# schmeing/ReSeq

Measured on AMD Instinct MI355X. Metric: simulated read-pairs/sec (2x150 bp), higher is better.
Workload: dtype f64

## Files before the change

### include/reseq_amd.h

```cpp
#ifndef RESEQ_AMD_H
#define RESEQ_AMD_H

#include <stddef.h>
#include <stdint.h>

#ifdef __cplusplus
extern "C" {
#endif

typedef struct rsq_profile rsq_profile;
typedef struct rsq_ref rsq_ref;
typedef struct rsq_sim rsq_sim;

enum {
    RSQ_OK = 0,
    RSQ_EINVAL = -1,
    RSQ_EIO = -2,
    RSQ_ENODEV = -3,
    RSQ_EHIP = -4,
    RSQ_ENOSPC = -5,
    RSQ_ESTATE = -6
};

const char *rsq_last_error(void);
const char *rsq_last_warning(void);
const char *rsq_version(void);
int rsq_set_option(const char *name, int64_t value);
int rsq_get_option(const char *name, int64_t *value);
int rsq_device_count(void);

int rsq_profile_load(const char *path, rsq_profile **out);
int rsq_profile_is_reseq_archive(const char *path, int *yes);
int rsq_profile_load_reseq(const char *stats_path, const char *ipf_path, double ipf_precision_percent, rsq_profile **out);
int rsq_profile_archive_layout(const char *stats_path, const char *ipf_path, char *out, size_t cap, size_t *need);
int rsq_profile_save(const rsq_profile *p, const char *path);
int rsq_profile_save_reseq(const rsq_profile *p, const char *stats_path, const char *ipf_path, uint64_t creation_time);
void rsq_profile_free(rsq_profile *p);
int rsq_profile_change_error_rate(rsq_profile *p, double error_multiplier);
int rsq_profile_remove_substitution_errors(rsq_profile *p);
int rsq_profile_remove_indel_errors(rsq_profile *p);
int rsq_profile_max_read_length(const rsq_profile *p, uint32_t *out);
int rsq_profile_num_tiles(const rsq_profile *p, uint32_t *out);
int rsq_profile_max_len_deletion(const rsq_profile *p, uint32_t *out);
int rsq_profile_ref_seq_bias(const rsq_profile *p, double *out, size_t cap, size_t *n);

int rsq_ref_load_fasta(const char *path, rsq_ref **out);
int rsq_ref_replace_n(rsq_ref *r, uint64_t seed);
void rsq_ref_free(rsq_ref *r);
int rsq_ref_num_sequences(const rsq_ref *r, uint32_t *out);
int rsq_ref_sequence_length(const rsq_ref *r, uint32_t seq, uint32_t *out);
int rsq_ref_sequence_name(const rsq_ref *r, uint32_t seq, char *out, size_t cap);
int rsq_ref_write_fasta(const rsq_ref *r, const char *path);
int rsq_ref_read_variants(rsq_ref *r, const char *path);
int rsq_ref_num_alleles(const rsq_ref *r, uint32_t *out);
int rsq_ref_num_variants(const rsq_ref *r, uint32_t seq, uint32_t *out);
int rsq_ref_get_variant(const rsq_ref *r, uint32_t seq, uint32_t index, uint32_t *position, char *var_seq, size_t var_seq_cap, uint64_t allele_bits[2]);
int rsq_ref_get_codes(const rsq_ref *r, uint32_t seq, uint8_t *out, uint32_t len);

int rsq_sim_create(const rsq_profile *p, const rsq_ref *ref, int device, rsq_sim **out);
void rsq_sim_free(rsq_sim *s);
int rsq_sim_take_options(rsq_sim *s);

int rsq_sim_reference_sequence(rsq_sim *s, uint32_t seq, uint32_t start_pos, uint32_t frag_length, int reversed, int32_t first_variant_id, uint32_t first_variant_pos, uint32_t allele,
                               uint8_t *out, size_t cap);

int rsq_sim_prepare(rsq_sim *s, uint64_t seed, uint64_t num_read_pairs, double coverage, int ref_bias_mode, const char *record_base_identifier, void *stream);

int rsq_sim_prepare_plan(rsq_sim *s, uint64_t seed, uint64_t num_read_pairs, double coverage, int ref_bias_mode, const char *record_base_identifier);
int rsq_sim_bias_partials(rsq_sim *s, uint32_t block_lo, uint32_t block_hi, double *sums, double *maxes, size_t cap, size_t *n, void *stream);
int rsq_sim_prepare_normalization(rsq_sim *s, const double *sums, const double *maxes, size_t n);
int rsq_sim_prepare_sys_errors(rsq_sim *s, uint32_t block_lo, uint32_t block_hi, const uint32_t in_state[2], uint32_t out_state[2], void *stream);
int rsq_sim_prepare_finish(rsq_sim *s);

int rsq_sim_read_methylation(rsq_sim *s, const char *path);

int rsq_sim_set_ref_bias_file(rsq_sim *s, const char *path);
int rsq_sim_get_ref_seq_bias(const rsq_sim *s, double *out, size_t n);

typedef struct {
    uint64_t total_pairs;
    uint64_t adapter_only_pairs;
    uint32_t total_blocks;
    uint32_t n_coverage_groups;
    uint32_t insert_to;
    uint32_t sys_chain_passes;
    double bias_normalization;
} rsq_sim_info;
int rsq_sim_get_info(const rsq_sim *s, rsq_sim_info *out);
int rsq_sim_get_fill_plan(const rsq_sim *s, uint32_t *quality_quads, uint32_t *image_tiles, uint32_t *image_bytes);
int rsq_sim_export_reference(rsq_sim *s, const char *path);
int rsq_sim_get_sequence_lengths(const rsq_sim *s, uint32_t *out, size_t cap, uint32_t *n_sequences);
int rsq_sim_import_reference(rsq_sim *s, const char *path);
int rsq_sim_specialize(rsq_sim *s, int kind, int *specialized);
int rsq_set_kernel_cache_dir(const char *path);
int rsq_profile_compile_read_kernel(const rsq_profile *p, int kind, int with_variants, int binned, const char *arch, const char *out_path, size_t *code_bytes, double *seconds);

int rsq_sim_get_thresholds(const rsq_sim *s, double *out, size_t n);
int rsq_sim_get_norm_by_len(const rsq_sim *s, double *out, size_t n);
int rsq_sim_set_normalization(rsq_sim *s, double bias_normalization, const double *thresholds, size_t n);
int rsq_sim_get_sys_errors(const rsq_sim *s, int reverse_strand, uint32_t seq, uint8_t *dom_out, uint8_t *rate_out, uint32_t len);
int rsq_sim_get_adapter_sys_errors(const rsq_sim *s, int template_segment, uint32_t adapter, uint8_t *dom_out, uint8_t *rate_out, uint32_t len);

int rsq_sim_create_sys_error_profile(rsq_sim *s, uint64_t seed, const char *path, void *stream);
int rsq_sim_read_sys_errors(rsq_sim *s, const char *path);

typedef struct {
    uint32_t seq, start, len;
    uint16_t dup;
    uint8_t strand, pad;
    uint32_t block, number;
} rsq_fragment;

int rsq_sim_block_weights(const rsq_sim *s, double *weights, size_t cap, uint32_t *n_blocks);
int rsq_partition_blocks(uint32_t total_blocks, uint32_t workers, const double *weights, uint32_t *bounds);

int rsq_sim_job_generate(rsq_sim *s, uint32_t block_lo, uint32_t block_hi, uint32_t batch_blocks, uint64_t *n_pairs, uint64_t *r1_bytes, uint64_t *r2_bytes, void *stream);
int rsq_sim_job_write(rsq_sim *s, const char *r1_path, uint64_t r1_offset, const char *r2_path, uint64_t r2_offset, uint32_t threads_per_file);
int rsq_sim_job_compress(rsq_sim *s, uint64_t *r1_bytes, uint64_t *r2_bytes);

size_t rsq_gzip_bound(size_t text_len);
size_t rsq_gzip_eof_member(char *out, size_t cap);
int rsq_sim_gzip_keep_code(rsq_sim *s, int keep);
int rsq_sim_gzip_device(rsq_sim *s, const char *text_dev, size_t text_len, char *out_dev, size_t out_cap, size_t *out_len, void *stream);
int rsq_sim_job_read(rsq_sim *s, int file, uint64_t at, size_t bytes, char *dst_dev, void *stream);
int rsq_sim_job_free(rsq_sim *s);
// ... 50 lines not shown
```

### reseq_amd/api.py

```python
import ctypes as C
import os

import numpy as np

_HERE = os.path.dirname(os.path.abspath(__file__))
LIB_PATH = os.path.join(_HERE, "libreseq_amd.so")

RSQ_OK, RSQ_EINVAL, RSQ_EIO, RSQ_ENODEV, RSQ_EHIP, RSQ_ENOSPC, RSQ_ESTATE = 0, -1, -2, -3, -4, -5, -6

FRAGMENT_DTYPE = np.dtype([("seq", "<u4"), ("start", "<u4"), ("len", "<u4"), ("dup", "<u2"), ("strand", "u1"),
                           ("allele", "u1"), ("block", "<u4"), ("number", "<u4")])


class SimInfo(C.Structure):
    _fields_ = [("total_pairs", C.c_uint64), ("adapter_only_pairs", C.c_uint64), ("total_blocks", C.c_uint32),
                ("n_coverage_groups", C.c_uint32), ("insert_to", C.c_uint32), ("sys_chain_passes", C.c_uint32),
                ("bias_normalization", C.c_double)]


class RsqError(RuntimeError):
    def __init__(self, code, message):
        super().__init__(f"rsq error {code}: {message}")
        self.code = code


_vp, _u64, _u32, _sz = C.c_void_p, C.c_uint64, C.c_uint32, C.c_size_t
_pp = C.POINTER(C.c_void_p)
_psz = C.POINTER(C.c_size_t)
SYMBOLS = {
    "rsq_last_error": (C.c_char_p, []),
    "rsq_version": (C.c_char_p, []),
    "rsq_set_option": (C.c_int, [C.c_char_p, C.c_int64]),
    "rsq_get_option": (C.c_int, [C.c_char_p, C.POINTER(C.c_int64)]),
    "rsq_device_count": (C.c_int, []),
    "rsq_profile_load": (C.c_int, [C.c_char_p, _pp]),
    "rsq_profile_load_reseq": (C.c_int, [C.c_char_p, C.c_char_p, C.c_double, _pp]),
    "rsq_profile_is_reseq_archive": (C.c_int, [C.c_char_p, C.POINTER(C.c_int)]),
    "rsq_profile_save": (C.c_int, [C.c_void_p, C.c_char_p]),
    "rsq_profile_save_reseq": (C.c_int, [C.c_void_p, C.c_char_p, C.c_char_p, C.c_uint64]),
    "rsq_profile_archive_layout": (C.c_int, [C.c_char_p, C.c_char_p, C.c_char_p, C.c_size_t, C.POINTER(C.c_size_t)]),
    "rsq_last_warning": (C.c_char_p, []),
    "rsq_profile_free": (None, [_vp]),
    "rsq_profile_change_error_rate": (C.c_int, [_vp, C.c_double]),
    "rsq_profile_remove_substitution_errors": (C.c_int, [_vp]),
    "rsq_profile_remove_indel_errors": (C.c_int, [_vp]),
    "rsq_profile_max_read_length": (C.c_int, [_vp, C.POINTER(_u32)]),
    "rsq_profile_num_tiles": (C.c_int, [_vp, C.POINTER(_u32)]),
    "rsq_profile_max_len_deletion": (C.c_int, [_vp, C.POINTER(_u32)]),
    "rsq_profile_ref_seq_bias": (C.c_int, [_vp, _vp, _sz, _psz]),
    "rsq_ref_sequence_name": (C.c_int, [_vp, _u32, C.c_char_p, _sz]),
    "rsq_ref_load_fasta": (C.c_int, [C.c_char_p, _pp]),
    "rsq_ref_replace_n": (C.c_int, [_vp, _u64]),
    "rsq_ref_free": (None, [_vp]),
    "rsq_ref_num_sequences": (C.c_int, [_vp, C.POINTER(_u32)]),
    "rsq_ref_sequence_length": (C.c_int, [_vp, _u32, C.POINTER(_u32)]),
    "rsq_ref_write_fasta": (C.c_int, [_vp, C.c_char_p]),
    "rsq_ref_read_variants": (C.c_int, [_vp, C.c_char_p]),
    "rsq_ref_num_alleles": (C.c_int, [_vp, C.POINTER(_u32)]),
    "rsq_ref_num_variants": (C.c_int, [_vp, _u32, C.POINTER(_u32)]),
    "rsq_ref_get_variant": (C.c_int, [_vp, _u32, _u32, C.POINTER(_u32), C.c_char_p, _sz, C.POINTER(_u64)]),
    "rsq_ref_get_codes": (C.c_int, [_vp, _u32, _vp, _u32]),
    "rsq_sim_create": (C.c_int, [_vp, _vp, C.c_int, _pp]),
    "rsq_sim_free": (None, [_vp]),
    "rsq_sim_take_options": (C.c_int, [_vp]),
    "rsq_sim_prepare": (C.c_int, [_vp, _u64, _u64, C.c_double, C.c_int, C.c_char_p, _vp]),
    "rsq_sim_prepare_plan": (C.c_int, [_vp, _u64, _u64, C.c_double, C.c_int, C.c_char_p]),
    "rsq_sim_bias_partials": (C.c_int, [_vp, _u32, _u32, _vp, _vp, C.c_size_t, C.POINTER(C.c_size_t), _vp]),
    "rsq_sim_prepare_normalization": (C.c_int, [_vp, _vp, _vp, C.c_size_t]),
    "rsq_sim_prepare_sys_errors": (C.c_int, [_vp, _u32, _u32, _vp, _vp, _vp]),
    "rsq_sim_prepare_finish": (C.c_int, [_vp]),
    "rsq_sim_get_info": (C.c_int, [_vp, C.POINTER(SimInfo)]),
    "rsq_sim_get_fill_plan": (C.c_int, [_vp, C.POINTER(_u32), C.POINTER(_u32), C.POINTER(_u32)]),
    "rsq_sim_specialize": (C.c_int, [_vp, C.c_int, C.POINTER(C.c_int)]),
    "rsq_sim_export_reference": (C.c_int, [_vp, C.c_char_p]),
    "rsq_sim_block_weights": (C.c_int, [_vp, _vp, _sz, C.POINTER(_u32)]),
    "rsq_partition_blocks": (C.c_int, [_u32, _u32, _vp, _vp]),
    "rsq_sim_reference_sequence": (C.c_int, [_vp, _u32, _u32, _u32, C.c_int, C.c_int32, _u32, _u32, _vp, _sz]),
    "rsq_sim_job_read": (C.c_int, [_vp, C.c_int, _u64, _sz, _vp, _vp]),
    "rsq_dev_pwrite": (C.c_int, [C.c_int, _vp, _sz, C.c_char_p, _u64]),
    "rsq_sim_get_sequence_lengths": (C.c_int, [_vp, _vp, _sz, C.POINTER(_u32)]),
    "rsq_sim_import_reference": (C.c_int, [_vp, C.c_char_p]),
    "rsq_set_kernel_cache_dir": (C.c_int, [C.c_char_p]),
    "rsq_profile_compile_read_kernel": (C.c_int, [_vp, C.c_int, C.c_int, C.c_int, C.c_char_p, C.c_char_p, C.POINTER(C.c_size_t), C.POINTER(C.c_double)]),
    "rsq_sim_get_thresholds": (C.c_int, [_vp, _vp, _sz]),
    "rsq_sim_get_norm_by_len": (C.c_int, [_vp, _vp, _sz]),
    "rsq_sim_set_normalization": (C.c_int, [_vp, C.c_double, _vp, _sz]),
    "rsq_sim_get_sys_errors": (C.c_int, [_vp, C.c_int, _u32, _vp, _vp, _u32]),
    "rsq_sim_get_adapter_sys_errors": (C.c_int, [_vp, C.c_int, _u32, _vp, _vp, _u32]),
    "rsq_sim_create_sys_error_profile": (C.c_int, [_vp, _u64, C.c_char_p, _vp]),
    "rsq_sim_read_sys_errors": (C.c_int, [_vp, C.c_char_p]),
    "rsq_sim_set_ref_bias_file": (C.c_int, [_vp, C.c_char_p]),
    "rsq_sim_read_methylation": (C.c_int, [_vp, C.c_char_p]),
    "rsq_sim_get_ref_seq_bias": (C.c_int, [_vp, _vp, _sz]),
    "rsq_sim_pairs": (C.c_int, [_vp, _u32, _u32, _vp, _sz, _psz, _vp, _sz, _psz, C.POINTER(_u64), _vp, _sz, _vp]),
    "rsq_sim_job_generate": (C.c_int, [_vp, _u32, _u32, _u32, C.POINTER(_u64), C.POINTER(_u64), C.POINTER(_u64), _vp]),
    "rsq_sim_job_write": (C.c_int, [_vp, C.c_char_p, _u64, C.c_char_p, _u64, _u32]),
    "rsq_sim_job_compress": (C.c_int, [_vp, C.POINTER(_u64), C.POINTER(_u64)]),
    "rsq_gzip_bound": (C.c_size_t, [C.c_size_t]),
    "rsq_gzip_eof_member": (C.c_size_t, [C.c_char_p, C.c_size_t]),
    "rsq_sim_gzip_keep_code": (C.c_int, [_vp, C.c_int]),
    "rsq_sim_gzip_device": (C.c_int, [_vp, _vp, C.c_size_t, _vp, C.c_size_t, C.POINTER(C.c_size_t), _vp]),
    "rsq_sim_job_free": (C.c_int, [_vp]),
    "rsq_sim_adapter_only_pairs": (C.c_int, [_vp, _u64, _u64, _vp, _sz, _psz, _vp, _sz, _psz, _vp]),
    "rsq_sim_error_model": (C.c_int, [_vp, _u64, _u64, _u32, _vp, _vp, _vp, _vp, _vp, _vp, _vp, _u32, _vp, _vp, _vp, _vp, _u32, _vp]),
    "rsq_sim_error_model_fastq": (C.c_int, [_vp, _u64, _u64, _u32, _vp, _vp, _vp, _vp, _vp, _vp, _vp, _vp, C.c_size_t, C.POINTER(C.c_size_t), _vp]),
    "rsq_sim_error_model_file": (C.c_int, [_vp, C.c_char_p, C.c_char_p, _vp, C.POINTER(_u64), C.POINTER(_u64)]),
    "rsq_fasta_count_records": (C.c_int, [C.c_char_p, _u64, _u64, _u32, C.POINTER(_u64), C.POINTER(_u64)]),
    "rsq_sim_error_model_fasta": (C.c_int, [_vp, _u64, _vp, C.c_size_t, C.c_int, _vp, C.c_size_t, C.POINTER(C.c_size_t), C.POINTER(_u64), C.POINTER(C.c_size_t), _vp]),
    "rsq_sim_last_kernel_ms": (C.c_int, [_vp, C.c_char_p, C.POINTER(C.c_double)]),
    "rsq_sim_last_kernel_launches": (C.c_int, [_vp, C.c_char_p, C.POINTER(_u32)]),
    "rsq_dev_alloc": (C.c_int, [C.c_int, _sz, _pp]),
    "rsq_dev_free": (C.c_int, [C.c_int, _vp]),
    "rsq_dev_upload": (C.c_int, [C.c_int, _vp, _vp, _sz]),
    "rsq_dev_download": (C.c_int, [C.c_int, _vp, _vp, _sz]),
    "rsq_host_alloc": (C.c_int, [_sz, _pp]),
    "rsq_host_free": (C.c_int, [_vp]),
    "rsq_stream_create": (C.c_int, [C.c_int, _pp]),
    "rsq_stream_destroy": (C.c_int, [C.c_int, _vp]),
    "rsq_dev_copy_on": (C.c_int, [C.c_int, _vp, _vp, _sz, C.c_int, _vp]),
}

_lib = None


def lib():
    global _lib
    if _lib is None:
        if not os.path.exists(LIB_PATH):
            raise ImportError(f"{LIB_PATH} is missing: build it with `python -c 'import __graft_entry__ as g; g.build()'` "
                              "(make -C reseq_amd/csrc); reseq_amd has no CPU fallback")
        L = C.CDLL(LIB_PATH)
        for name, (res, args) in SYMBOLS.items():
            fn = getattr(L, name)
            fn.restype = res
            fn.argtypes = args
        _lib = L
    return _lib


def use_library(path):
    global LIB_PATH, _lib
    if _lib is not None:
        raise RuntimeError("the library is already loaded")
    LIB_PATH = os.path.abspath(path)


def set_option(name, value):
    _check(lib().rsq_set_option(name.encode(), int(value)))


def get_option(name):
    v = C.c_int64(0)
    _check(lib().rsq_get_option(name.encode(), C.byref(v)))
    return v.value


def archive_layout(stats_path, ipf_path=None):
    need = C.c_size_t(0)
    ipf = ipf_path.encode() if ipf_path else None
    _check(lib().rsq_profile_archive_layout(str(stats_path).encode(), ipf, None, 0, C.byref(need)))
    buf = C.create_string_buffer(need.value)
    _check(lib().rsq_profile_archive_layout(str(stats_path).encode(), ipf, buf, need.value, C.byref(need)))
    return buf.value.decode(errors="replace")


def gzip_eof_member():
    buf = C.create_string_buffer(32)
    n = lib().rsq_gzip_eof_member(buf, 32)
    return buf.raw[:n]


def partition_blocks(total_blocks, workers, weights=None):
    w = np.ascontiguousarray(np.ones(total_blocks) if weights is None else weights, dtype=np.float64)
    if w.size != total_blocks:
        raise ValueError("one weight per block")
    bounds = np.zeros(workers + 1, np.uint32)
    _check(lib().rsq_partition_blocks(total_blocks, workers, w.ctypes.data, bounds.ctypes.data))
    return [(int(bounds[r]), int(bounds[r + 1])) for r in range(workers)]


def dev_pwrite(device, src_ptr, nbytes, path, offset):
    _check(lib().rsq_dev_pwrite(device, C.c_void_p(src_ptr), nbytes, os.fsencode(path), offset))


def set_kernel_cache_dir(path):
    _check(lib().rsq_set_kernel_cache_dir((path or "").encode()))


def last_warning():
    return lib().rsq_last_warning().decode(errors="replace")


def _check(rc):
    if rc != RSQ_OK:
        raise RsqError(rc, lib().rsq_last_error().decode(errors="replace"))


def device_count():
    n = lib().rsq_device_count()
    if n < 0:
        raise RsqError(n, lib().rsq_last_error().decode())
    return n


class Profile:

    def __init__(self, path, ipf_path=None, ipf_precision=5.0):
        self.h = C.c_void_p()
        if ipf_path is None and ipf_precision == 5.0:
            _check(lib().rsq_profile_load(os.fsencode(path), C.byref(self.h)))
        else:
            _check(lib().rsq_profile_load_reseq(os.fsencode(path), os.fsencode(ipf_path) if ipf_path else None, ipf_precision, C.byref(self.h)))
        self.warning = lib().rsq_last_warning().decode()

    def save(self, path):
        _check(lib().rsq_profile_save(self.h, os.fsencode(path)))

    def save_reseq(self, stats_path, ipf_path=None, creation_time=0):
        _check(lib().rsq_profile_save_reseq(self.h, os.fsencode(stats_path), os.fsencode(ipf_path) if ipf_path else None, int(creation_time)))

    def compile_read_kernel(self, kind=0, with_variants=False, binned=False, arch="gfx950", out_path=None):
        n, t = C.c_size_t(0), C.c_double(0.0)
        _check(lib().rsq_profile_compile_read_kernel(self.h, kind, int(with_variants), int(binned), arch.encode(), os.fsencode(out_path) if out_path else None, C.byref(n), C.byref(t)))
        return n.value, t.value

    def change_error_rate(self, multiplier):
        _check(lib().rsq_profile_change_error_rate(self.h, multiplier))

    def remove_substitution_errors(self):
        _check(lib().rsq_profile_remove_substitution_errors(self.h))

    def remove_indel_errors(self):
        _check(lib().rsq_profile_remove_indel_errors(self.h))

    def max_read_length(self):
        v = C.c_uint32()
        _check(lib().rsq_profile_max_read_length(self.h, C.byref(v)))
        return v.value

    def close(self):
        if self.h:
            lib().rsq_profile_free(self.h)
            self.h = C.c_void_p()


def load_profile(path, ipf_path=None, ipf_precision=5.0):
    archive = C.c_int(0)
    lib().rsq_profile_is_reseq_archive(os.fsencode(path), C.byref(archive))
    if not archive.value:
        return Profile(path)
    p = Profile.__new__(Profile)
    p.h = C.c_void_p()
    _check(lib().rsq_profile_load_reseq(os.fsencode(path), os.fsencode(ipf_path) if ipf_path else None, float(ipf_precision), C.byref(p.h)))
    p.warning = lib().rsq_last_warning().decode()
    return p


class Reference:

    def __init__(self, fasta_path, replace_n_seed=None):
        self.h = C.c_void_p()
        _check(lib().rsq_ref_load_fasta(os.fsencode(fasta_path), C.byref(self.h)))
        if replace_n_seed is not None:
            _check(lib().rsq_ref_replace_n(self.h, replace_n_seed))

    def num_sequences(self):
        v = C.c_uint32()
        _check(lib().rsq_ref_num_sequences(self.h, C.byref(v)))
        return v.value

    def sequence_length(self, i):
        v = C.c_uint32()
        _check(lib().rsq_ref_sequence_length(self.h, i, C.byref(v)))
        return v.value

    def sequence_name(self, i):
        buf = C.create_string_buffer(1 << 16)
        _check(lib().rsq_ref_sequence_name(self.h, i, buf, len(buf)))
        return buf.value.decode()

    def read_variants(self, path):
        _check(lib().rsq_ref_read_variants(self.h, str(path).encode()))
        n = _u32()
        _check(lib().rsq_ref_num_alleles(self.h, C.byref(n)))
        return n.value

    def variants(self, seq):
        n = _u32()
        _check(lib().rsq_ref_num_variants(self.h, seq, C.byref(n)))
        out = []
        for i in range(n.value):
            pos, buf, bits = _u32(), C.create_string_buffer(1 << 16), (_u64 * 2)()
            _check(lib().rsq_ref_get_variant(self.h, seq, i, C.byref(pos), buf, len(buf), bits))
            out.append((pos.value, buf.value.decode(), bits[0] | (bits[1] << 64)))
        return out

    def write_fasta(self, path):
        _check(lib().rsq_ref_write_fasta(self.h, str(path).encode()))

    def codes(self, i):
        out = np.zeros(self.sequence_length(i), np.uint8)
        _check(lib().rsq_ref_get_codes(self.h, i, out.ctypes.data, len(out)))
        return out

    def close(self):
        if self.h:
            lib().rsq_ref_free(self.h)
            self.h = C.c_void_p()


class ErrorModelFileOptions(C.Structure):
    _fields_ = [("read_threads", C.c_uint32), ("block_kb", C.c_uint32), ("batch_blocks", C.c_uint32), ("keep_text", C.c_uint32), ("from_", C.c_uint64), ("to", C.c_uint64), ("first_record", C.c_uint64),
                ("progress", C.c_void_p), ("user", C.c_void_p), ("trace", C.c_char_p), ("trace_cap", C.c_size_t)]


def count_fasta_records(path, from_=0, to=0, threads=0):
    n, first = _u64(0), _u64(0)
    _check(lib().rsq_fasta_count_records(os.fsencode(path), from_, to, threads, C.byref(n), C.byref(first)))
    return n.value, first.value


class DeviceArray:

    def __init__(self, device, nbytes):
        self.device, self.nbytes = device, int(nbytes)
        self.ptr = C.c_void_p()
# ... 319 lines not shown
```

### reseq_amd/csrc/rsq_core.h

```cpp
#pragma once
#include "rsq_types.h"
#if !defined(__HIPCC_RTC__)
#include <math.h>
#endif

namespace rsq {

struct Words {
    uint32_t w0, w1, w2, w3;
};


RSQ_HD Words philox(uint64_t seed, uint32_t c0, uint32_t c1, uint32_t c2, uint32_t c3) {
    uint32_t k0 = (uint32_t)seed, k1 = (uint32_t)(seed >> 32);
#pragma unroll
    for (int r = 0; r < 10; ++r) {
        const uint64_t p0 = (uint64_t)0xD2511F53u * c0, p1 = (uint64_t)0xCD9E8D57u * c2;
        const uint32_t hi0 = (uint32_t)(p0 >> 32), lo0 = (uint32_t)p0, hi1 = (uint32_t)(p1 >> 32), lo1 = (uint32_t)p1;
        c0 = hi1 ^ c1 ^ k0;
        c1 = lo1;
        c2 = hi0 ^ c3 ^ k1;
        c3 = lo0;
        k0 += 0x9E3779B9u;
        k1 += 0xBB67AE85u;
// ... 620 lines not shown

    template <class Tab, class Src, class Out>
    RSQ_HD bool step(const DevSim &S, const Tab &tab, const Stream &st, const Src &src, Out &out) {
        if (!advance(S, st)) return false;
        iterate(S, tab, st, src, out);
        return true;
    }
    RSQ_HD bool in_template() const { return phase == kTemplate && par.read_pos < par.read_length && org_pos < org_len; }
    template <bool TEMPLATE_PART = false, class Tab, class Src, class Out>
    RSQ_HD void iterate(const DevSim &S, const Tab &tab, const Stream &st, const Src &src, Out &out) {
        const bool tail = !TEMPLATE_PART && phase == kTail, from_template = TEMPLATE_PART || phase == kTemplate;
        const DevAdapters &ad = S.adapters[seg];
        const uint32_t it = par.iteration;
        const Words w = st.step(2u + it);
        typename Tab::Sum prob_sum;
        uint32_t indel = 0, org_base = 0;
        if (!tail) {
            const uint32_t idx_i[3] = {par.indel_pos, par.read_pos, par.gc_seq};
            indel = tab.draw_indel(par.previous_indel_type * 6u + par.base_call, idx_i, w.w0, prob_sum);
            if (0 == prob_sum) indel = 0;
            org_base = from_template ? src.base(org_pos) : (uint32_t)ad.seqs[adapter_a0 + org_pos];
        }
        const uint32_t qi = tbase + org_base;
        const bool regular = !tail && 0 == indel, deletion = !tail && 1 == indel;
        uint32_t dom_error = 0;
        if (regular) {
            const uint32_t se = from_template ? src.sys_base(org_pos) : (uint32_t)ad.sys[adapter_a0 + org_pos];
            dom_error = se & 0xFFu;
            par.error_rate = se >> 8;
        } else if (deletion) {
            par.error_rate = (from_template ? src.sys_deleted(org_pos) : (uint32_t)ad.sys[adapter_a0 + org_pos]) >> 8;
        }
        uint32_t q = 0;
        if (!deletion) {
            const uint32_t idx_q[4] = {par.seq_qual, par.qual, par.read_pos, par.error_rate};
            q = tab.draw_quality(qi, idx_q, w.w1, prob_sum);
            if (0 == prob_sum) {
                if (regular) q = par.read_pos ? par.last_written_qual : tab.quality(qi).max_value;
                else if (tail) q = par.read_pos ? par.last_written_qual : q;
                else q = par.qual;
            }
        }
        uint32_t put_base = 0, op_code = 0;
        char element = 0;
        const bool insertion = !tail && indel > 1u;
        if (regular) {
            par.qual = q;
            const uint32_t idx_b[4] = {par.qual, par.read_pos, par.num_errors, par.error_rate};
            uint32_t call = tab.draw_base_call(qi * 5u + dom_error, idx_b, w.w2, prob_sum);
            if (0 == prob_sum) call = org_base;
            par.base_call = call;
            put_base = call;
            element = from_template ? 'M' : 'S';
            if (call != org_base) ++par.num_errors;
        } else if (deletion) {
            op_code = 1u;
            element = 'D';
        } else if (tail) {
            par.qual = q;
            put_base = pos_tail < tail_length ? 0u : discrete_draw(S.overrun_cp, 4, u32_to_unit(w.w3));
            ++pos_tail;
        } else {
            put_base = indel - 2u;
            op_code = 2u;
            element = 'I';
        }
        if (element) {
            const uint32_t is_indel = deletion || insertion ? 1u : 0u;
            n_indels += is_indel;
            par.num_errors += is_indel;
            if (element == cg.element) {
                ++cg.length;
                par.indel_pos += is_indel;
            } else {
                cg.flush();
                cg.element = element;
                cg.length = 1;
                par.indel_pos = is_indel;
                par.previous_indel_type = deletion ? 1u : 0u;
            }
            if (!insertion) ++org_pos;
        }
        if (!deletion) {
            out.put(par.read_pos, put_base, q + RSQ_SIM(S, phred_offset));
            par.last_written_qual = q;
            ++par.read_pos;
        }
        if (!tail) out.op(it, op_code);
        par.iteration = it + 1u;
    }

    RSQ_HD void finalize(ReadMeta &meta) const {
        meta.read_len = (uint16_t)par.read_length;
        meta.num_errors = (uint16_t)par.num_errors;
        meta.n_iter_m = (uint16_t)iter_m;
        meta.n_iter_s = (uint16_t)(par.iteration - iter_m - hard_clip);
        meta.hard_clip = (uint16_t)hard_clip;
        meta.tile_id = (uint16_t)tile_id;
        meta.cigar_chars = (uint16_t)cg.chars;
        meta.plain = n_indels ? 0u : 1u;
    }
};

template <class Tab, class Src, class Out>
RSQ_HD void fill_read(const DevSim &S, const Tab &tab, const Stream &st, uint32_t seg, uint32_t tile_id, uint32_t fragment_length, const Src &src, Out &out,
                      ReadMeta &meta) {
    ReadMachine m;
    m.init(S, tab, st, seg, tile_id, fragment_length, src);
    while (m.step(S, tab, st, src, out)) {}
    m.finalize(meta);
}

}
```

### reseq_amd/csrc/rsq_format.h

```cpp
#pragma once
#include "rsq_reads.h"

namespace rsq {

#if RSQ_DEVICE_BUILD
#ifndef RSQ_BIN_KEYS_LDS
#define RSQ_BIN_KEYS_LDS 4096
#endif
constexpr uint32_t kBinKeysLds = RSQ_BIN_KEYS_LDS;
constexpr uint32_t kBinItemsPerThread = 16, kBinBlock = 256;

__device__ inline void bin_count_key(uint32_t key, bool valid, uint32_t n_keys, uint32_t *hist, uint32_t *s_hist) {
    if (n_keys <= kBinKeysLds) {
        for (uint32_t k = threadIdx.x; k < n_keys; k += blockDim.x) s_hist[k] = 0;
        __syncthreads();
        if (valid) atomicAdd(&s_hist[key], 1u);
        __syncthreads();
        for (uint32_t k = threadIdx.x; k < n_keys; k += blockDim.x)
            if (s_hist[k]) atomicAdd(&hist[k], s_hist[k]);
    } else if (valid) atomicAdd(&hist[key], 1u);
}
__global__ void __launch_bounds__(kBinBlock) k_pair_tiles(DevSim S, const Fragment *frags, const FragmentVar *fvars, uint64_t n_pairs, uint64_t adapter_only_first, uint16_t *key_of,
                                                         uint32_t *hist) {
    __shared__ uint32_t s_hist[kBinKeysLds];
// ... 96 lines not shown
    const uint64_t i = (uint64_t)blockIdx.x * blockDim.x + threadIdx.x;
    if (i >= n) return;
    const uint32_t seg = segs[i] ? 1u : 0u, fl = frag_len[i];
    if (fl < range.lo[seg] || fl >= range.hi[seg]) atomicMin(first_bad, (uint32_t)i);
}
__global__ void k_record_flags(const uint8_t *segs, uint64_t n, uint32_t *flags) {
    const uint64_t i = (uint64_t)blockIdx.x * blockDim.x + threadIdx.x;
    if (i < n) flags[i] = segs[i] ? 1u : 0u;
}
__global__ void k_record_partition(const uint8_t *segs, uint64_t n, const uint64_t *ones_before, uint32_t *rec_index, uint32_t *rec_count) {
    const uint64_t i = (uint64_t)blockIdx.x * blockDim.x + threadIdx.x;
    const uint32_t n1 = (uint32_t)ones_before[n], n0 = (uint32_t)n - n1;
    if (i == 0) {
        rec_count[0] = n0;
        rec_count[1] = n1;
    }
    if (i >= n) return;
    const uint32_t before = (uint32_t)ones_before[i];
    if (segs[i]) rec_index[n0 + before] = (uint32_t)i;
    else rec_index[(uint32_t)i - before] = (uint32_t)i;
}

__global__ void __launch_bounds__(256) k_methylation_templates(DevSim S, const Fragment *frags, uint64_t n_pairs, RawLayout raw) {
    const uint64_t r = (uint64_t)blockIdx.x * blockDim.x + threadIdx.x;
    if (r >= 2u * n_pairs) return;
    const uint32_t seg = r >= n_pairs ? 1u : 0u;
    convert_template(S, frags[r - seg * n_pairs], seg, raw.templates + r * raw.template_words, raw.template_words);
}

__global__ void __launch_bounds__(256) k_variant_templates(DevSim S, const Fragment *frags, const FragmentVar *fvars, uint64_t n_pairs, RawLayout raw) {
    const uint64_t r = (uint64_t)blockIdx.x * blockDim.x + threadIdx.x;
    if (r >= 2u * n_pairs) return;
    const uint32_t seg = r >= n_pairs ? 1u : 0u;
    const uint64_t pair = r - seg * n_pairs;
    variant_template(S, frags[pair], fvars[pair], seg, raw.templates + r * raw.template_words, raw.template_words);
}

#ifndef RSQ_FORMAT_RECORDS
#define RSQ_FORMAT_RECORDS 16
#endif
constexpr uint32_t kFormatRecords = RSQ_FORMAT_RECORDS, kFormatLdsMax = 16u * 1024u, kFormatLdsMin = 1024u;
RSQ_HD uint32_t format_lds_bytes(uint64_t record_bytes) {
    const uint64_t want = (kFormatRecords * record_bytes + 16u + 127u) & ~(uint64_t)127u;
    return (uint32_t)(want < kFormatLdsMin ? kFormatLdsMin : want > kFormatLdsMax ? kFormatLdsMax : want);
}
__global__ void __launch_bounds__(256) k_max_size(const uint32_t *sizes, uint64_t n, uint32_t *longest) {
    uint32_t m = 0;
    for (uint64_t i = (uint64_t)blockIdx.x * blockDim.x + threadIdx.x; i < n; i += (uint64_t)gridDim.x * blockDim.x) m = max(m, sizes[i]);
    for (uint32_t d = 32; d; d >>= 1) m = max(m, (uint32_t)__shfl_xor((int)m, (int)d, 64));
    if ((threadIdx.x & 63u) == 0 && m) atomicMax(longest, m);
}
template <bool PERM>
__global__ void __launch_bounds__(64) k_format_write(DevSim S, NameTable names, const Fragment *frags, uint64_t n_pairs, uint64_t adapter_only_first, RawLayout raw,
                                                    const uint64_t *offsets0, const uint64_t *offsets1, char *dst0, char *dst1, uint64_t cap0, uint64_t cap1,
                                                    const FragmentVar *fvars, const uint32_t *perm, uint32_t lds_bytes) {
    extern __shared__ __attribute__((aligned(16))) char s_text[];
    const uint32_t lane = threadIdx.x, seg = blockIdx.y, rec = lane & (kFormatRecords - 1u), part = lane / kFormatRecords;
    constexpr uint32_t kLineParts = 32u / kFormatRecords;
    const bool is_qual = part >= kLineParts;
    const uint32_t sub = part % kLineParts;
    const uint64_t first = (uint64_t)blockIdx.x * kFormatRecords;
    if (first >= n_pairs) return;
    const uint64_t *offsets = seg ? offsets1 : offsets0;
    char *dst = seg ? dst1 : dst0;
    if (offsets[n_pairs] > (seg ? cap1 : cap0)) return;
    const uint64_t last = first + kFormatRecords < n_pairs ? first + kFormatRecords : n_pairs;
    const uint64_t row = first + rec;
    const bool active = row < last;
    const uint64_t pair = PERM ? (active ? perm[row] : 0u) : row;
    const uint64_t g_begin = PERM ? (active ? offsets[pair] : 0u) : offsets[first], g_end = PERM ? (active ? offsets[pair + 1u] : 0u) : offsets[last];
    const uint32_t skew = (uint32_t)((uint64_t)(uintptr_t)(dst + g_begin) & 15u), bytes = (uint32_t)(g_end - g_begin);
    const uint32_t kSlot = (lds_bytes / kFormatRecords) & ~15u;
    const bool through_lds = PERM ? __all(skew + bytes <= kSlot) != 0 : skew + bytes <= lds_bytes;
    ReadMeta m;
    Fragment f;
    FragmentVar fv;
    uint64_t r = 0;
    if (active) {
        r = (uint64_t)seg * n_pairs + row;
        m = raw.meta[r];
        if (frags) f = frags[pair];
        if (frags && fvars) fv = fvars[pair];
    }
    const WordColumn seq = raw.seq_of(r), qual = raw.qual_of(r), ops = raw.ops_of(r);
    const uint64_t ao_number = adapter_only_first + pair + 1u;
    if (!through_lds) {
        if (active && part == 0u) format_record(S, names, frags != nullptr, f, ao_number, m, seq, qual, ops, dst + offsets[pair], frags && fvars, fv);
        return;
    }
    const uint32_t slot_at = PERM ? rec * kSlot : 0u;
    if (active) {
        RSQ_LDS char *rec_text = (RSQ_LDS char *)s_text + slot_at + skew + (PERM ? 0u : (uint32_t)(offsets[pair] - g_begin));
        const uint32_t header = (uint32_t)(offsets[pair + 1u] - offsets[pair]) - 2u * m.read_len - 4u;
        const uint32_t all_words = (m.read_len + 3u) >> 2, per = (all_words + kLineParts - 1u) / kLineParts;
        const uint32_t first_word = sub * per, line_at = header + (is_qual ? m.read_len + 3u : 0u);
        const uint32_t part_at = part == 0u ? 0u : line_at + (4u * first_word < m.read_len ? 4u * first_word : m.read_len);
        WordSinkT<RSQ_LDS char *> t(rec_text + part_at);
        if (part == 0u) format_header(S, names, frags != nullptr, f, ao_number, m, ops, t, frags && fvars, fv);
        format_line_part(is_qual ? qual : seq, m.read_len, is_qual, first_word, per, sub == kLineParts - 1u, t);
        t.finish();
    }
    __syncthreads();
    const uint32_t lo = skew, hi = skew + bytes;
    char *g_chunk0 = dst + g_begin - skew;
    const char *s_from = s_text + slot_at;
    for (uint32_t c = (PERM ? part : lane) * 16u; c < hi; c += (PERM ? 64u / kFormatRecords : 64u) * 16u) {
        if (c >= lo && c + 16u <= hi) {
            *reinterpret_cast<uint4 *>(g_chunk0 + c) = *reinterpret_cast<const uint4 *>(s_from + c);
        } else {
            for (uint32_t b = c < lo ? lo : c; b < c + 16u && b < hi; ++b) g_chunk0[b] = s_from[b];
        }
    }
}

#endif

}
```

### reseq_amd/csrc/rsq_pack.h

```cpp
#pragma once
#include <math.h>
#include <stdio.h>
#include <stdlib.h>
#include <string.h>
#include <errno.h>
#include <fcntl.h>
#include <unistd.h>

#include <algorithm>
#include <string>
#include <vector>

#include <atomic>
#include <exception>
#include <mutex>
#include <thread>

#include "rsq_host.h"
#include "rsq_chains.h"
#include "rsq_sieve.h"
#include "rsq_reads.h"

namespace rsq {

// ... 339 lines not shown
        auto need_rate = [&](uint32_t rows_q, uint32_t rows_b) {
            return (uint64_t)4 * Ti * odd_stride((uint64_t)rows_q * plan.slot_q) + (uint64_t)20 * Ti * odd_stride((uint64_t)rows_b * plan.slot_b);
        };
        const uint32_t ring_stride = 4 * Ti * plan.slot_q;
        need += (uint64_t)kFillWavesMax * kRingRows * ring_stride;
        if (need + need_rate(1, 1) > budget) return false;
        uint32_t rq = 1, rb = 1;
        while (rq < std::min(rate_rows_q, kLdsRateRowsFirst) && need + need_rate(rq + 1, 1) <= budget) ++rq;
        const bool stage_b2 = need + need_b2 + need_rate(rq, 1) <= budget;
        if (stage_b2) need += need_b2;
        const bool stage_i0 = need + need_i0 + need_rate(rq, 1) <= budget;
        if (stage_i0) need += need_i0;
        while (rb < std::min(rate_rows_b, kLdsRateRowsFirst) && need + need_rate(rq, rb + 1) <= budget) ++rb;
        while (rq < rate_rows_q && need + need_rate(rq + 1, rb) <= budget) ++rq;
        while (rb < rate_rows_b && need + need_rate(rq, rb + 1) <= budget) ++rb;
        plan.img_tiles = Ti;
        plan.binned = (Ti < T || opt.image_tiles == 1) ? 1u : 0u;
        plan.par0_words = par0_words;
        plan.par0_indel_bytes = par0_indel_bytes;
        plan.desc_words = desc_words;
        plan.ring_stride = ring_stride;
        plan.rate_rows_q = rq;
        plan.rate_rows_b = rb;
        plan.q.values = desc_words * 4u;
        plan.b.values = plan.q.values + 4 * Ti * plan.slot_q;
        plan.i.values = plan.b.values + 20 * Ti * plan.slot_b;
        uint32_t at = desc_words + values_words;
        plan.q.lds = at, plan.q.lds_rows = rows_q, plan.q.lds_stride = stride_q, at += (uint32_t)need_q;
        plan.b.lds = at, plan.b.lds_rows = rows_b, plan.b.lds_stride = stride_b, at += (uint32_t)need_b;
        plan.b.lds2 = stage_b2 ? at : kNoLds;
        plan.b.lds2_stride = stride_b2;
        if (stage_b2) at += (uint32_t)need_b2;
        plan.i.lds = stage_i0 ? at : kNoLds;
        plan.i.lds_rows = rows_i;
        plan.i.lds_stride = stride_i;
        if (stage_i0) at += (uint32_t)need_i0;
        plan.ring_off = at;
        plan.q3_off = plan.ring_off + kFillWavesMax * kRingRows * plan.ring_stride;
        plan.q3_stride = odd_stride((uint64_t)plan.rate_rows_q * plan.slot_q);
        plan.b3_stride = odd_stride((uint64_t)plan.rate_rows_b * plan.slot_b);
        plan.b3_off = plan.q3_off + 4 * Ti * plan.q3_stride;
        plan.total_words = plan.b3_off + 20 * Ti * plan.b3_stride;
        plan.mask = plan.quads_q;
        return true;
    };
    plan.img_tiles = T;
    if (screenable && opt.fill_mode != 0) {
        const bool per_tile_first = opt.image_tiles == 1 && T > 1;
        if (!(per_tile_first && plan_image(1)) && !plan_image(T) && !(T > 1 && plan_image(1)))
            s.plan_note = "the read kernels' table image does not fit the " + std::to_string(kLdsBudgetBytes / 1024u) +
                          " KiB of local memory even for one tile: every per-base draw runs in double precision from device memory (several times slower)";
    } else if (!screenable && opt.fill_mode != 0)
        s.plan_note = "the profile's tables are outside what the screened single-precision draws are built for (more than " + std::to_string(4u * kQualityQuads[4]) +
                      " quality values, or more than 8 base-call / indel outcomes): every per-base draw runs in double precision from device memory (several times slower)";
    if ((plan.desc_words | plan.q3_off | plan.b3_off | plan.ring_off | plan.ring_stride | plan.slot_q | plan.slot_b | plan.slot_i | plan.q.off32 | plan.b.off32 | plan.i.off32 |
         (plan.mask ? plan.q.lds | plan.b.lds | (plan.b.lds2 != kNoLds ? plan.b.lds2 : 0u) | (plan.i.lds != kNoLds ? plan.i.lds : 0u) : 0u)) & 3u)
        throw Error("internal: LDS rows must start on 16-byte boundaries");
    if (opt.trace_plan)
        fprintf(stderr, "[rsq] LDS image: mask %u, %u of %u tiles per image, %u words (%u KiB), desc %u, quality slot %u, rate rows %u / %u, q3 %u b3 %u, ring %u x %u, b2 %d i0 %d\n", plan.mask,
                plan.img_tiles, T, plan.total_words, plan.total_words / 256, plan.desc_words, plan.slot_q, plan.rate_rows_q, plan.rate_rows_b, plan.q3_off, plan.b3_off, plan.ring_off,
                plan.ring_stride, (int)(plan.b.lds2 != kNoLds), (int)(plan.i.lds != kNoLds));
    s.dev.lds = plan;
    s.dev.quality = up.put(quality);
    s.dev.seq_quality = up.put(seq_quality);
    s.dev.base_call = up.put(base_call);
    s.dev.dom_error = up.put(dom_error);
    s.dev.error_rate = up.put(error_rate);
    s.dev.indels = up.put(indels);
    par0.resize(((par0.size() + 3u) & ~(size_t)3u) + (size_t)plan.par0_words * 4u + 16u, 0);
    pool.push_back(0.0);
    pool.push_back(0.0);
    pool32.resize(pool32.size() + 8, 0.f);
    s.dev.pool = up.put(pool);
    s.dev.pool32 = up.put(pool32);
    s.dev.par0 = up.put(par0);
    s.host_pool = pool;
    s.host_par0 = par0;
    s.host_dom_error = dom_error;
    s.host_error_rate = error_rate;
}

inline uint32_t effective_fill_mask(uint32_t plan_mask, int forced) { return forced == 0 ? 0u : plan_mask; }

inline void pack_profile(SimState &s, Uploader &up) {
    const Profile &p = s.prof;
    DevSim &d = s.dev;
    d.n_tiles = p.n_tiles();
    d.phred_offset = p.phred_offset;
    d.max_len_deletion = p.max_len_deletion;
    d.reset_distance = p.reset_distance;
    d.tile_cp = up.put(discrete_cp(p.tile_abundance.data(), p.tile_abundance.size()));
    d.tiles = up.put(p.tiles);
    s.rmax = 0;
    uint32_t max_adapter = 0;
    for (int seg = 0; seg < 2; ++seg) {
        const HostAdapters &a = p.adapters[seg];
        DevAdapters &da = d.adapters[seg];
        da.n = a.n();
        da.seqs = up.put(a.seqs);
        da.seq_ptr = up.put(a.seq_ptr);
        da.adapter_cp = up.put(discrete_cp(a.significant.data(), a.significant.size()));
        std::vector<double> cut_cp;
        for (uint32_t i = 0; i < a.n(); ++i) {
            std::vector<double> cp = discrete_cp(a.cut.data() + a.cut_ptr[i], a.cut_ptr[i + 1] - a.cut_ptr[i]);
            cp.resize(a.cut_ptr[i + 1] - a.cut_ptr[i]);
            cut_cp.insert(cut_cp.end(), cp.begin(), cp.end());
            max_adapter = std::max(max_adapter, a.seq_ptr[i + 1] - a.seq_ptr[i]);
        }
        cut_cp.push_back(1.0);
        da.cut_cp = up.put(cut_cp);
        da.cut_ptr = up.put(a.cut_ptr);
        da.cut_from = up.put(a.cut_from);
        s.adapter_sys[seg] = up.put(std::vector<uint16_t>(a.seqs.size() + 1, 0));
        da.sys = s.adapter_sys[seg];

        const Vect<uint64_t> &rl = p.read_lengths[seg];
        DevReadLengths &dr = d.read_lengths[seg];
        if (rl.v.empty()) throw Error("profile has no read lengths");
        dr.fixed = rl.v.size() == 1 ? (uint32_t)rl.from : 0u;
        dr.to = (uint32_t)rl.to();
        dr.row_first = (uint32_t)p.rl_by_fl[seg].from;
        dr.rows = (uint32_t)p.rl_by_fl[seg].row_ptr.size() - 1;
        dr.row_ptr = up.put(p.rl_by_fl[seg].row_ptr);
        dr.row_from = up.put(p.rl_by_fl[seg].row_from);
        dr.values = up.put(p.rl_by_fl[seg].values);
        s.rmax = std::max(s.rmax, dr.to - 1);
    }
    d.polya_cp = up.put(discrete_cp(p.polya.v.data(), p.polya.v.size()));
    d.polya_n = (uint32_t)p.polya.v.size();
    d.polya_from = (uint32_t)p.polya.from;
    std::vector<double> ocp = discrete_cp(p.overrun_bases, 4);
    for (int i = 0; i < 4; ++i) d.overrun_cp[i] = ocp[i];
    d.insert_from = (uint32_t)std::max<uint64_t>(1, p.insert_lengths.from);
    s.insert_lengths_from = p.insert_lengths.from;
    if (p.insert_lengths.to() > 65536) throw Error("insert lengths above 65535 are not supported (fragment lengths are 16-bit fields of the sieve's records)");
    d.insert_to = (uint32_t)p.insert_lengths.to();
    std::vector<uint64_t> il(d.insert_to + 1, 0);
    std::vector<double> ilb(d.insert_to + 1, 0.0), gcb(101, 0.0);
    for (uint32_t i = 0; i < d.insert_to; ++i) {
        il[i] = p.insert_lengths[i];
        ilb[i] = p.insert_lengths_bias[i];
    }
    for (uint32_t i = 0; i < 101; ++i) gcb[i] = p.gc_bias[i];
    d.insert_lengths = up.put(il);
    d.insert_lengths_bias = up.put(ilb);
    d.gc_bias = up.put(gcb);
    d.sur_bias = up.put(p.sur_bias);
    d.dispersion[0] = p.dispersion[0];
    d.dispersion[1] = p.dispersion[1];

    s.max_adapter = max_adapter;
    s.read_stride = (s.rmax + 15u) & ~15u;
    const uint32_t max_iter = 2u * s.rmax + p.max_len_deletion + max_adapter + 4u;
    s.ops_stride = (max_iter + 15u) / 16u;
}

inline int variants_mode_for(const Variants &v) {
    if (v.num_alleles > kMaxDevAlleles) throw Error("variants: more than " + std::to_string(kMaxDevAlleles) + " alleles");
    if (v.num_alleles > 8) return 2;
    for (const std::vector<Variant> &seq : v.by_seq)
        for (const Variant &x : seq)
            if (x.var_seq.size() != 1) return 2;
    return 1;
}

inline void allele_maps_of_sequence(const std::vector<Variant> &vars, const std::vector<uint8_t> &codes, uint32_t num_alleles, const std::string &name,
                                    std::vector<AlleleVar> &out, std::vector<uint32_t> &ptr) {
    auto is_gc_code = [](uint8_t c) { return c == 1 || c == 2; };
    for (uint32_t a = 0; a < num_alleles; ++a) {
        int32_t shift = 0, gc = 0;
        int64_t last_pos = -1;
// ... 1202 lines not shown
```

### reseq_amd/csrc/rsq_reads.h

```cpp
#pragma once
#include "rsq_core.h"
#include "rsq_variants.h"
#include "rsq_text.h"

namespace rsq {

struct ReadOut {
    WordColumn seq, qual, ops;
    uint32_t cur_word, cur_index;
    uint32_t seq_word, qual_word, n_put;
    RSQ_HD void put(uint32_t pos, uint32_t base, uint32_t qual_char) {
        const uint32_t sh = (pos & 3u) * 8u;
        seq_word |= base << sh;
        qual_word |= qual_char << sh;
        n_put = pos + 1u;
        if ((pos & 3u) == 3u) {
            seq.at(pos >> 2) = seq_word;
            qual.at(pos >> 2) = qual_word;
            seq_word = qual_word = 0;
        }
    }
    RSQ_HD void op(uint32_t it, uint32_t code) {
        const uint32_t wi = it >> 4;
        if (wi != cur_index) {
            ops.at(cur_index) = cur_word;
            cur_word = 0;
            cur_index = wi;
        }
        cur_word |= code << ((it & 15u) * 2u);
    }
    RSQ_HD void finish() {
        ops.at(cur_index) = cur_word;
        if (n_put & 3u) {
            seq.at(n_put >> 2) = seq_word;
            qual.at(n_put >> 2) = qual_word;
        }
    }
};
RSQ_HD ReadOut make_read_out(const WordColumn &seq, const WordColumn &qual, const WordColumn &ops) { return ReadOut{seq, qual, ops, 0u, 0u, 0u, 0u, 0u}; }

struct RawLayout {
    uint32_t *seq, *qual;
    uint32_t *ops;
    ReadMeta *meta;
    uint64_t pitch;
    uint64_t *templates;
    uint32_t template_words;
    const uint32_t *order;
    RSQ_HD uint64_t item_of(uint64_t row) const { return order ? order[row] : row; }
    RSQ_HD WordColumn seq_of(uint64_t r) const { return WordColumn{seq + r, pitch}; }
    RSQ_HD WordColumn qual_of(uint64_t r) const { return WordColumn{qual + r, pitch}; }
    RSQ_HD WordColumn ops_of(uint64_t r) const { return WordColumn{ops + r, pitch}; }
    RSQ_HD ReadOut out_of(uint64_t r) const { return make_read_out(seq_of(r), qual_of(r), ops_of(r)); }
};

struct FragmentSrc {
    const uint64_t *words;
    uint64_t word_off;
    uint32_t first;
    uint32_t len;
    bool reverse;
    const uint16_t *sys_;
    const uint64_t *converted;
    const uint32_t *gc_prefix;
    mutable uint32_t held_word = 0xFFFFFFFFu, held_sys = 0xFFFFFFFFu;
    mutable uint64_t word = 0, sys4 = 0;
    RSQ_HD uint64_t template_word(const uint64_t *from, uint32_t index) const {
        if (index != held_word) {
            held_word = index;
            word = from[index];
        }
        return word;
    }
    RSQ_HD uint32_t org_len() const { return len; }
    RSQ_HD uint32_t ref(uint32_t k) const {
        const uint32_t pos = reverse ? first - 1u - k : first + k, b = (uint32_t)(template_word(words + word_off, pos >> 5) >> ((pos & 31u) * 2u)) & 3u;
        return reverse ? 3u - b : b;
    }
    RSQ_HD uint32_t base(uint32_t k) const { return converted ? (uint32_t)(template_word(converted, k >> 5) >> ((k & 31u) * 2u)) & 3u : ref(k); }
    RSQ_HD uint32_t sys_base(uint32_t k) const {
        if ((k >> 2) != held_sys) {
            held_sys = k >> 2;
#if defined(__HIP_DEVICE_COMPILE__)
            sys4 = *reinterpret_cast<const uint64_t __attribute__((aligned(2))) *>(sys_ + (k & ~3u));
#else
            memcpy(&sys4, sys_ + (k & ~3u), 8);
#endif
        }
        return (uint32_t)(sys4 >> ((k & 3u) * 16u)) & 0xFFFFu;
    }
    RSQ_HD uint32_t sys_deleted(uint32_t k) const { return sys_base(k); }
    RSQ_HD void totals(uint32_t n, uint32_t &gc, uint32_t &rate_sum) const {
        if (!converted && !gc_prefix) return template_totals_loop(*this, n, gc, rate_sum);
        if (converted) gc += ref_gc_count(converted, 0, 0, n);
        else gc += reverse ? ref_gc_count_prefix(words, gc_prefix, word_off, first - n, first) : ref_gc_count_prefix(words, gc_prefix, word_off, first, first + n);
        rate_sum += rate_total(n);
    }
    RSQ_HD uint32_t rate_total(uint32_t n) const {
        struct __attribute__((packed, aligned(2))) Eight {
            uint64_t a, b;
        };
        uint32_t sum = 0;
        for (uint32_t k = 0; k < n; k += 8u) {
            Eight e;
#if defined(__HIP_DEVICE_COMPILE__)
            e = *reinterpret_cast<const Eight *>(sys_ + k);
#else
            memcpy(&e, sys_ + k, 16);
#endif
            const uint32_t left = n - k;
            if (left < 8u) {
                if (left <= 4u) {
                    e.b = 0;
                    if (left < 4u) e.a &= (1ull << (16u * left)) - 1ull;
                } else e.b &= (1ull << (16u * (left - 4u))) - 1ull;
            }
            const uint64_t kHigh = 0x00FF00FF00FF00FFull, kAdd = 0x0001000100010001ull;
            sum += (uint32_t)((((e.a >> 8) & kHigh) * kAdd) >> 48) + (uint32_t)((((e.b >> 8) & kHigh) * kAdd) >> 48);
        }
        return sum;
    }
};

struct MethView {
    const uint32_t *first, *second;
    const double *rate;
    uint32_t n, stride;
    RSQ_HD double rate_of(int32_t region) const { return rate[(size_t)region * stride]; }
};
RSQ_HD MethView meth_view(const DevSim &S, uint32_t seq, uint32_t allele = 0) {
    const uint32_t off = S.meth_ptr[seq];
    return MethView{S.meth_first + off, S.meth_second + off, S.meth_rate + (size_t)off * S.num_alleles + allele, S.meth_ptr[seq + 1] - off, S.num_alleles};
}
RSQ_HD uint32_t meth_start_index(const MethView &m, uint32_t pos) {
    uint32_t lo = 0, hi = m.n;
    while (lo < hi) {
// ... 669 lines not shown
struct FillBins {
    const uint32_t *perm;
    const uint32_t *bin_first;
    const uint32_t *bin_count;
    const uint32_t *chunk_ptr;
    uint32_t *next_chunk;
    uint32_t *workers;
    uint32_t n_bins;
    const Fragment *frags;
    const FragmentVar *fvars;
};
constexpr uint32_t kSchedWords = 8;

struct PairStream {
    uint32_t c0, c1, c2, strand;
};
RSQ_HD PairStream pair_stream(const Fragment *f, uint32_t sub, uint64_t adapter_only_number) {
    if (f) return PairStream{f->start, f->seq | (sub << 22), f->len | ((uint32_t)f->dup << 16), f->strand};
    return PairStream{(uint32_t)adapter_only_number, 0xFFFFFFFFu, (uint32_t)(adapter_only_number >> 32), 0u};
}

#if RSQ_DEVICE_BUILD
template <uint32_t MASK>
__device__ RSQ_LDS float *fill_stage_image(const DevSim &S, float *lds_image, uint32_t qbase) {
    RSQ_LDS float *img = (RSQ_LDS float *)lds_image;
    if (MASK) {
        lds_stage_descriptors(S, img, qbase, threadIdx.x, blockDim.x);
        __syncthreads();
        lds_stage_rows(S, img, qbase, threadIdx.x, blockDim.x);
        __syncthreads();
    }
    return img;
}
template <uint32_t MASK, class Src>
__device__ void fill_wave_reads(const DevSim &S, RSQ_LDS float *img, uint32_t qbase, uint32_t seg, bool active, const Stream &st, uint32_t tile, uint32_t fragment_length,
                                const Src &src, ReadOut &out, ReadMeta &meta) {
    ReadMachine m;
    if constexpr (MASK == 0) {
        const GlobalTables tab{S};
        if (active) {
            m.init(S, tab, st, seg, tile, fragment_length, src);
            while (m.step(S, tab, st, src, out)) {}
        }
    } else {
        const uint32_t lane = threadIdx.x & 63u, n_items = lds_ring_items(S);
        RSQ_LDS float *ring = img + RSQ_PLAN(S, ring_off) + (threadIdx.x >> 6) * kRingRows * RSQ_PLAN(S, ring_stride);
        ScreenTables<MASK> tab{S, img, qbase, ring, 0u};
        m.idle();
        if (active) m.init(S, tab, st, seg, tile, fragment_length, src);
        const RingItem mine = lds_ring_item(S, qbase, lane < n_items ? lane : 0u);
        Quad ahead = lane < n_items ? lds_ring_load(S, mine, 0u) : zero_quad();
        auto begin_step = [&](uint32_t t) {
            if (lane < n_items) {
                lds_ring_store(S, mine, ring, t, ahead);
                ahead = lds_ring_load(S, mine, t + 1u);
            }
            for (uint32_t item = lane + 64u; item < n_items; item += 64u) lds_ring_stage(S, qbase, ring, t, item);
            __builtin_amdgcn_wave_barrier();
            tab.t = t;
            const uint64_t lagging = __builtin_amdgcn_ballot_w64(m.phase != ReadMachine::kDone && t - m.par.read_pos > kRingLag);
            tab.demand = 0xFFFFFFFFu;
            if (lagging) {
                const uint32_t p = __builtin_amdgcn_readlane(m.par.read_pos, __builtin_ctzll(lagging));
                if (lane < n_items) lds_ring_stage_demand(S, mine, ring, p);
                for (uint32_t item = lane + 64u; item < n_items; item += 64u) lds_ring_stage_demand(S, lds_ring_item(S, qbase, item), ring, p);
                __builtin_amdgcn_wave_barrier();
                tab.demand = p;
            }
        };
        uint32_t t = 0;
        for (; !RSQ_ANY(!m.in_template()); ++t) {
            begin_step(t);
            m.template iterate<true>(S, tab, st, src, out);
            __builtin_amdgcn_wave_barrier();
        }
        for (; RSQ_ANY(m.phase != ReadMachine::kDone); ++t) {
            begin_step(t);
            m.step(S, tab, st, src, out);
            __builtin_amdgcn_wave_barrier();
        }
    }
    if (active) {
        m.finalize(meta);
        out.finish();
    }
}

template <uint32_t MASK, class Chunk>
__device__ void fill_binned_loop(const DevSim &S, float *lds_image, const FillBins &bins, Chunk &&chunk) {
    RSQ_LDS float *img = (RSQ_LDS float *)lds_image;
    RSQ_LDS uint32_t *sched = reinterpret_cast<RSQ_LDS uint32_t *>(img + (MASK ? RSQ_PLAN(S, total_words) : 0u));
    const uint32_t lane = threadIdx.x & 63u;
    if (threadIdx.x == 0) sched[1] = 0xFFFFFFFFu;
    for (bool first_choice = true;; first_choice = false) {
        if (threadIdx.x < 64u) {
            uint64_t best = 0;
            if (first_choice) {
                const uint64_t total = bins.chunk_ptr[bins.n_bins], target = ((2u * (uint64_t)blockIdx.x + 1u) * total) / (2u * gridDim.x);
                uint32_t lo = 0, hi = bins.n_bins;
                while (hi - lo > 1u) {
                    const uint32_t mid = (lo + hi) >> 1;
                    if (bins.chunk_ptr[mid] <= target) lo = mid;
                    else hi = mid;
                }
                best = total ? ((uint64_t)1 << 32) | (0xFFFFFFFFu - lo) : 0u;
            } else {
                for (uint32_t b = lane; b < bins.n_bins; b += 64u) {
                    const uint32_t n = (bins.bin_count[b] + 63u) / 64u, done = __hip_atomic_load(&bins.next_chunk[b], __ATOMIC_RELAXED, __HIP_MEMORY_SCOPE_AGENT),
                                   on_it = __hip_atomic_load(&bins.workers[b], __ATOMIC_RELAXED, __HIP_MEMORY_SCOPE_AGENT), left = done < n ? n - done : 0u;
                    const uint64_t score = (uint64_t)left * 4096u / (on_it + 1u), packed = (score << 32) | (0xFFFFFFFFu - b);
                    if (left && packed > best) best = packed;
                }
            }
            for (uint32_t d = 32; d; d >>= 1) {
                const uint64_t other = ((uint64_t)(uint32_t)__shfl_xor((int)(best >> 32), (int)d, 64) << 32) | (uint32_t)__shfl_xor((int)(uint32_t)best, (int)d, 64);
                best = other > best ? other : best;
            }
            if (lane == 0) {
                const uint32_t bin = best ? 0xFFFFFFFFu - (uint32_t)best : 0xFFFFFFFFu;
                sched[0] = bin;
                if (best) atomicAdd(&bins.workers[bin], 1u);
            }
        }
        __syncthreads();
        const uint32_t bin = (uint32_t)__builtin_amdgcn_readfirstlane((int)sched[0]);
        if (bin == 0xFFFFFFFFu) break;
        const uint32_t seg = bin / RSQ_SIM(S, n_tiles), tile = bin - seg * RSQ_SIM(S, n_tiles), qbase = image_qbase(S, seg, tile);
        if (bin != (uint32_t)__builtin_amdgcn_readfirstlane((int)sched[1])) {
            fill_stage_image<MASK>(S, lds_image, qbase);
            if (threadIdx.x == 0) sched[1] = bin;
        }
        const uint32_t first = bins.bin_first[bin], n_items = bins.bin_count[bin];
        for (;;) {
            uint32_t c = 0;
            if (lane == 0) c = atomicAdd(&bins.next_chunk[bin], 1u);
            c = (uint32_t)__builtin_amdgcn_readfirstlane((int)c);
            if ((uint64_t)c * 64u >= n_items) break;
            chunk(img, qbase, seg, tile, first + c * 64u, c * 64u + lane < n_items);
        }
        __syncthreads();
        if (threadIdx.x == 0) atomicSub(&bins.workers[bin], 1u);
    }
}

template <uint32_t MASK, bool VAR, bool BINNED>
__device__ void fill_pair_chunk(const DevSim &S, const NameTable &names, RSQ_LDS float *img, uint32_t qbase, uint32_t seg, uint32_t bin_tile, uint64_t row, bool active,
                                const Fragment *frags, uint64_t n_pairs, uint64_t adapter_only_first, const RawLayout &raw, uint32_t *sizes, const FragmentVar *fvars,
                                const uint32_t *perm) {
    const uint64_t at = active ? row : 0u, r_out = (uint64_t)seg * n_pairs + at;
    ReadOut out = raw.out_of(r_out);
    Fragment f{};
    if (active && frags) f = frags[at];
    const bool from_fragment = frags != nullptr;
    FragmentVar fv{};
    if (VAR && active && fvars) fv = fvars[at];
    const bool need_pair = !from_fragment || raw.templates != nullptr;
    const uint64_t pair0 = BINNED ? (need_pair && active ? perm[at] : 0u) : at;
    const PairStream ps = pair_stream(from_fragment ? &f : nullptr, fv.sub, adapter_only_first + pair0);
    const Stream st{S.seed, ps.c0, ps.c1, ps.c2, pair_c3(kDomPair, ps.strand, seg, f.allele)};
    const uint32_t tile = BINNED ? bin_tile : (active ? draw_tile(S, ps.c0, ps.c1, ps.c2, pair_c3(kDomPair, ps.strand, 2, f.allele)) : 0u);
    ReadMeta meta;
    if constexpr (VAR) {
        VariantSrc src = variant_src(S, f, fvars ? &fv : nullptr, seg);
        if (raw.templates) src.converted = raw.templates + ((uint64_t)seg * n_pairs + pair0) * raw.template_words;
        fill_wave_reads<MASK>(S, img, qbase, seg, active, st, tile, f.len, src, out, meta);
    } else {
        FragmentSrc src = from_fragment && active ? fragment_src(S, f, seg) : FragmentSrc{S.ref_words, 0, 0, 0, false, S.sys_fwd, nullptr, nullptr};
// ... 115 lines not shown
```

### reseq_amd/csrc/rsq_sim.hip

```cpp
#include <hip/hip_runtime.h>
#include <fcntl.h>
#include <sys/mman.h>
#include <sys/stat.h>
#include <math.h>
#include <string.h>
#include <unistd.h>

#include <algorithm>
#include <atomic>
#include <chrono>
#include <map>
#include <thread>
#include <memory>
#include <string>
#include <utility>
#include <vector>

#include "../../include/reseq_amd.h"
#include "rsq_deflate.h"
#include "rsq_fasta.h"
#include "rsq_chains.h"
#include "rsq_sieve.h"
#include "rsq_scan.h"
#include "rsq_text.h"
// ... 86 lines not shown
        HIP_CHECK(hipEventRecord(events[used].second, st));
        ++used;
    }
    double ms() const {
        double sum = 0.0;
        for (size_t i = 0; i < used; ++i) {
            float t = 0;
            if (hipEventElapsedTime(&t, events[i].first, events[i].second) == hipSuccess) sum += t;
        }
        return sum;
    }
    size_t launches() const { return used; }
};

}

using namespace rsq;

struct rsq_profile {
    Profile p;
};
struct rsq_ref {
    Reference r;
    Variants variants;
    bool has_variants = false;
};

struct DeviceUploader : Uploader {
    std::vector<std::unique_ptr<DevBuf>> owned[kUploadScopes];
    int device = 0;
    void bind_thread() override { HIP_CHECK(hipSetDevice(device)); }
    void release_scope(int scope) override {
        HIP_CHECK(hipDeviceSynchronize());
        owned[scope].clear();
    }
    void *put_bytes(const void *data, size_t bytes) override {
        std::vector<std::unique_ptr<DevBuf>> &own = owned[current_scope];
        own.emplace_back(new DevBuf());
        own.back()->reserve(bytes + 8);
        HIP_CHECK(hipMemcpy(own.back()->as<void>(), data, bytes, hipMemcpyHostToDevice));
        return own.back()->as<void>();
    }
    void *put_zeros(size_t bytes) override {
        std::vector<std::unique_ptr<DevBuf>> &own = owned[current_scope];
        own.emplace_back(new DevBuf());
        own.back()->reserve(bytes + 8);
        HIP_CHECK(hipMemset(own.back()->as<void>(), 0, bytes + 8));
        return own.back()->as<void>();
    }
    void write_bytes(void *dst, const void *src, size_t bytes) override { HIP_CHECK(hipMemcpy(dst, src, bytes, hipMemcpyHostToDevice)); }
    void read_bytes(void *dst_host, const void *src, size_t bytes) override { HIP_CHECK(hipMemcpy(dst_host, src, bytes, hipMemcpyDeviceToHost)); }
};

struct MappedFile {
    const char *data = nullptr;
    size_t size = 0;
    explicit MappedFile(const char *path) {
        const int fd = open(path, O_RDONLY);
        if (fd < 0) throw Error(std::string("cannot open ") + path + ": " + strerror(errno));
        struct stat st;
        if (fstat(fd, &st) != 0 || st.st_size <= 0) {
            close(fd);
            throw Error(std::string(path) + " is empty or cannot be examined");
        }
        size = (size_t)st.st_size;
        void *p = mmap(nullptr, size, PROT_READ, MAP_PRIVATE, fd, 0);
        close(fd);
        if (p == MAP_FAILED) throw Error(std::string("cannot map ") + path);
        data = static_cast<const char *>(p);
    }
    ~MappedFile() {
        if (data) munmap(const_cast<char *>(data), size);
    }
    MappedFile(const MappedFile &) = delete;
    MappedFile &operator=(const MappedFile &) = delete;
};

struct rsq_sim : SimState {
    int device = 0;
    DeviceUploader up;
    struct Workspace {
        DevBuf fvars;
        DevBuf slot_table;
        DevBuf counts, offsets, tile_sums, scan_total, frags, raw_seq, raw_qual, raw_ops, raw_meta, sizes, off_r1, off_r2, fill_counters, hits, hit_count, cands, pairs_of, pair_off, templates, rec_flags, rec_index, rec_count;
        DevBuf bin_keys, bin_small, bin_perm, bin_frags, bin_fvars;
        DevBuf fa_counts, fa_first, fa_at, fa_len, fa_id_len, fa_frag_len, fa_seg, fa_codes, fa_summary;
        DevBuf cell_info;
        hipEvent_t text_done = nullptr;
    } ws[2];
    struct JobText {
        std::vector<std::unique_ptr<DevBuf>> chunks[2];
        std::vector<size_t> used[2];
        uint64_t bytes[2] = {0, 0};
        bool complete = false;
        std::vector<unsigned char> packed[2];
        bool is_packed = false;
        bool device_packed = false;
        void clear() {
            complete = false;
            is_packed = false;
            device_packed = false;
            for (auto &p : packed) std::vector<unsigned char>().swap(p);
            for (int f = 0; f < 2; ++f) {
                chunks[f].clear();
                used[f].clear();
                bytes[f] = 0;
            }
        }
    } job;
    DevBuf totals;
    bool gz_dense = false;
    bool gz_keep_code = false, gz_have_code = false;
    DevBuf gz_slots, gz_sizes, gz_at, gz_hist, gz_codes, gz_total;
    Workspace *cur = &ws[0];
    hipStream_t side[2] = {nullptr, nullptr};
    hipEvent_t ev_call = nullptr, ev_fill = nullptr, ev_emit = nullptr;
    std::map<std::string, Timer> timers;
    uint32_t n_cu = 256;
    uint64_t *mailbox = nullptr;
    uint64_t format_record_bytes = 480;
    DevBuf longest_record;
    uint64_t record_text_bytes = 480;
    int force_fill_mode = -1;
    SpecKernels spec;
    std::string arch;
    bool specialize = true;
    BiasPlan bias_plan;
    bool planned = false;
    struct ChainRun {
        std::vector<Chain> chains;
        ShardEdges edges;
        uint32_t n_chunks = 0, passes = 0, block_lo = 0, block_hi = 0;
        bool pass_through = false;
        DevBuf d_chains, d_chunk_chain, d_used, d_out[2], d_changed, d_list;
        bool valid = false;
    } chain_run;
};

static bool fill_is_binned(const rsq_sim &s) { return effective_fill_mask(s.dev.lds.mask, s.force_fill_mode) != 0 && s.dev.lds.binned; }
static thread_local std::string g_spec_note;
static hipFunction_t spec_kernel(rsq_sim &s, SpecKind kind, uint32_t mask, bool var, bool binned) {
    if (!s.specialize || mask == 0) return nullptr;
    std::string note;
    hipFunction_t fn = s.spec.get(s.dev, SpecVariant{kind, mask, var, binned}, s.arch, note);
    if (s.opt.trace_plan && note != g_spec_note) fprintf(stderr, "[rsq] %s\n", note.c_str());
    g_spec_note = note;
    return fn;
}

namespace rsq {

static void iterate_sys_chains(rsq_sim &s, rsq_sim::ChainRun &run, hipStream_t st, uint32_t first_pass) {
    run.d_list.reserve((size_t)run.n_chunks * 4 + 16);
    uint32_t pass = first_pass;
    for (;; ++pass) {
        uint32_t *out_prev = run.d_out[(pass + 1) & 1].as<uint32_t>(), *out_new = run.d_out[pass & 1].as<uint32_t>();
        uint32_t n_run = run.n_chunks;
        const uint32_t *list = nullptr;
        if (pass > 0) {
            HIP_CHECK(hipMemsetAsync(run.d_changed.as<uint32_t>(), 0, 4, st));
            hipLaunchKernelGGL(k_sys_chain_select, dim3(cdiv(run.n_chunks, 256)), dim3(256), 0, st, run.d_chains.as<Chain>(), run.d_chunk_chain.as<uint32_t>(), run.n_chunks,
                               run.d_used.as<uint32_t>(), out_prev, out_new, run.d_list.as<uint32_t>(), run.d_changed.as<uint32_t>(), (int)pass);
            HIP_CHECK(hipGetLastError());
            HIP_CHECK(hipMemcpyAsync(&n_run, run.d_changed.as<uint32_t>(), 4, hipMemcpyDeviceToHost, st));
            HIP_CHECK(hipStreamSynchronize(st));
            list = run.d_list.as<uint32_t>();
        }
// ... 91 lines not shown
                           d_start_bias.as<double>(), d_end_bias.as<double>(), a, d_sum.as<double>(), d_max.as<double>(), a, b);
        HIP_CHECK(hipGetLastError());
    }
    lap("track and sum kernels");
    HIP_CHECK(hipMemcpyAsync(h_sum.data(), d_sum.as<double>(), h_sum.size() * 8, hipMemcpyDeviceToHost, st));
    HIP_CHECK(hipMemcpyAsync(h_max.data(), d_max.as<double>(), h_max.size() * 8, hipMemcpyDeviceToHost, st));
    HIP_CHECK(hipStreamSynchronize(st));
    lap("download");
}
static void bias_normalization(rsq_sim &s, hipStream_t st) {
    const BiasPlan plan = plan_bias_normalization(s, s.up);
    std::vector<double> h_sum, h_max;
    bias_partials(s, st, plan, 0, UINT64_MAX, h_sum, h_max);
    normalization_from_partials(s, s.up, plan, h_sum.data(), h_max.data());
}

static void prepare(rsq_sim &s, uint64_t seed, uint64_t num_read_pairs, double coverage, int ref_bias_mode, const char *base_identifier, hipStream_t st) {
    HIP_CHECK(hipSetDevice(s.device));
    const bool trace = s.opt.trace_prepare != 0;
    auto now = [] { return std::chrono::steady_clock::now(); };
    auto lap = [&](const char *what, std::chrono::steady_clock::time_point &t0) {
        if (trace) fprintf(stderr, "prepare: %-28s %8.3f s\n", what, std::chrono::duration<double>(now() - t0).count());
        t0 = now();
    };
    auto t0 = now();
    plan_simulation(s, s.up, seed, num_read_pairs, coverage, ref_bias_mode, base_identifier);
    lap("plan", t0);
    s.planned = false;
    if (s.has_ref) {
        bias_normalization(s, st);
        lap("bias normalisation", t0);
    }
    s.passes = run_sys_chains(s, st, s.has_ref ? kChainsSimulation : kChainsAdapters);
    HIP_CHECK(hipStreamSynchronize(st));
    lap("systematic-error chains", t0);
    if (s.has_variants && s.chain_run.valid) variant_sys_errors_from_run(s, st);
    lap("variants' systematic errors", t0);
    s.prepared = true;
    s.prepared_lo = 1;
    s.prepared_hi = s.total_blocks + 1;
    if (s.has_ref) (void)spec_kernel(s, SpecKind::kReads, effective_fill_mask(s.dev.lds.mask, s.force_fill_mode), s.has_variants, fill_is_binned(s));
    lap("read kernel for the profile", t0);
}

static void create_sys_error_profile(rsq_sim &s, uint64_t seed, const char *path, hipStream_t st) {
    if (!s.has_ref) throw Error("a reference is needed to draw a systematic error profile");
    HIP_CHECK(hipSetDevice(s.device));
    s.dev.seed = seed;
    set_sys_gc_range(s);
    run_sys_chains(s, st, kChainsProfile);
    s.prepared = false;
    std::string text;
    std::vector<uint16_t> track;
    std::vector<uint8_t> dom, rate;
    for (uint32_t i = 0; i < s.dev.n_seqs; ++i)
        for (uint32_t strand = 2; strand--;) {
            const uint32_t L = s.seq_len[i];
            track.resize(L);
            dom.resize(L);
            rate.resize(L);
            HIP_CHECK(hipMemcpy(track.data(), (strand ? s.sys_rev : s.sys_fwd) + s.seq_base_off[i], (size_t)L * 2, hipMemcpyDeviceToHost));
            for (uint32_t k = 0; k < L; ++k) {
                dom[k] = (uint8_t)(track[k] & 0xFF);
                rate[k] = (uint8_t)(track[k] >> 8);
            }
            text += sys_error_fastq_record(s.ref_ids[i] + (strand ? " reverse" : " forward"), dom.data(), rate.data(), L);
        }
    write_text_file(path, text);
}

static void exclusive_scan(rsq_sim &s, const uint32_t *in, uint64_t n, uint64_t *out, hipStream_t st, const uint64_t *init = nullptr, uint64_t *total_out = nullptr) {
    const uint32_t tiles = cdiv(n, kScanTile);
    s.cur->tile_sums.reserve((size_t)(tiles + 1) * 8);
    s.cur->scan_total.reserve(8);
    uint64_t *total = total_out ? total_out : s.cur->scan_total.as<uint64_t>();
    hipLaunchKernelGGL(k_scan_tile_sums, dim3(tiles), dim3(kScanBlock), 0, st, in, n, s.cur->tile_sums.as<uint64_t>());
    hipLaunchKernelGGL(k_scan_tiles, dim3(1), dim3(kScanTilesBlock), 0, st, s.cur->tile_sums.as<uint64_t>(), tiles, total, init);
    hipLaunchKernelGGL(k_scan_apply, dim3(tiles), dim3(kScanBlock), 0, st, in, n, s.cur->tile_sums.as<uint64_t>(), total, out);
    HIP_CHECK(hipGetLastError());
}

static RawLayout raw_layout(rsq_sim &s, uint64_t n_reads) {
    const uint64_t pitch = (n_reads + 63u) & ~(uint64_t)63u;
    s.cur->raw_seq.reserve((uint64_t)(s.read_stride / 4u) * pitch * 4 + 16);
    s.cur->raw_qual.reserve((uint64_t)(s.read_stride / 4u) * pitch * 4 + 16);
    s.cur->raw_ops.reserve((uint64_t)s.ops_stride * pitch * 4 + 16);
    s.cur->raw_meta.reserve(n_reads * sizeof(ReadMeta) + 16);
    return RawLayout{s.cur->raw_seq.as<uint32_t>(), s.cur->raw_qual.as<uint32_t>(), s.cur->raw_ops.as<uint32_t>(), s.cur->raw_meta.as<ReadMeta>(), pitch, nullptr, 0, nullptr};
}

template <class CountKernel>
static FillBins build_fill_bins(rsq_sim &s, uint64_t n_items, uint32_t n_keys, hipStream_t st, CountKernel &&count_keys, const Fragment *frags = nullptr,
                                const FragmentVar *fvars = nullptr) {
    if (n_items >= 0xFFFFFFFFull) throw Error("more than 2^32 reads in one call of a profile with tiles: use smaller block ranges");
    const uint32_t n_bins = 2 * s.dev.n_tiles;
    s.cur->bin_keys.reserve(n_items * 2 + 16);
    s.cur->bin_perm.reserve(n_items * 4 + 16);
    const size_t words = 2 * (size_t)n_keys + 5 * (size_t)n_bins + 1;
    s.cur->bin_small.reserve(words * 4 + 16);
    uint32_t *hist = s.cur->bin_small.as<uint32_t>(), *cursor = hist + n_keys, *bin_first = cursor + n_keys, *bin_count = bin_first + n_bins, *next_chunk = bin_count + n_bins,
             *workers = next_chunk + n_bins, *chunk_ptr = workers + n_bins;
    HIP_CHECK(hipMemsetAsync(hist, 0, (size_t)n_keys * 4, st));
    s.timers["bin_tiles"].start(st);
    count_keys(s.cur->bin_keys.as<uint16_t>(), hist);
    hipLaunchKernelGGL(k_bins_plan, dim3(1), dim3(1024), 0, st, hist, n_keys, n_bins, bin_first, bin_count, cursor, chunk_ptr, next_chunk, workers);
    if (frags) s.cur->bin_frags.reserve(n_items * sizeof(Fragment) + 16);
    if (fvars) s.cur->bin_fvars.reserve(n_items * sizeof(FragmentVar) + 16);
    hipLaunchKernelGGL(k_bin_scatter, dim3(cdiv(n_items, kBinBlock * kBinItemsPerThread)), dim3(kBinBlock), 0, st, s.cur->bin_keys.as<uint16_t>(), n_items, n_keys, cursor,
                       s.cur->bin_perm.as<uint32_t>(), frags, fvars, s.cur->bin_frags.as<Fragment>(), s.cur->bin_fvars.as<FragmentVar>());
    s.timers["bin_tiles"].stop(st);
    HIP_CHECK(hipGetLastError());
    return FillBins{s.cur->bin_perm.as<uint32_t>(), bin_first, bin_count, chunk_ptr, next_chunk, workers, n_bins, s.cur->bin_frags.as<Fragment>(), s.cur->bin_fvars.as<FragmentVar>()};
}
static void spec_allow_lds(hipFunction_t fn, size_t lds_bytes) {
    if (lds_bytes > 64 * 1024 && hipFuncSetAttribute(reinterpret_cast<const void *>(fn), hipFuncAttributeMaxDynamicSharedMemorySize, (int)lds_bytes) != hipSuccess) (void)hipGetLastError();
}
template <class Kernel>
static size_t fill_lds_bytes(const rsq_sim &s, bool screened, bool binned, Kernel kernel) {
    const size_t lds_bytes = (screened ? (size_t)s.dev.lds.total_words * 4u : 0) + (binned ? kSchedWords * 4u : 0);
    if (lds_bytes > 64 * 1024) HIP_CHECK(hipFuncSetAttribute(reinterpret_cast<const void *>(kernel), hipFuncAttributeMaxDynamicSharedMemorySize, (int)lds_bytes));
    return lds_bytes;
}
struct FillShape {
    uint32_t blocks, threads;
};
static FillShape fill_shape(const rsq_sim &s, size_t lds_bytes, uint64_t n_items, uint32_t segments_per_item, uint32_t max_threads) {
    const uint32_t per_cu = lds_bytes * 2 <= kLdsBudgetBytes ? 2u : 1u;
    const uint64_t chunks = segments_per_item * ((n_items + 63) / 64), slots = (uint64_t)s.n_cu * per_cu;
    uint32_t waves = (uint32_t)std::min<uint64_t>(max_threads / 64u, std::max<uint64_t>(4u, cdiv(chunks, slots)));
    waves = std::min(max_threads / 64u, (waves + 3u) & ~3u);
    if (s.opt.fill_waves > 0) waves = (uint32_t)std::min<int64_t>(max_threads / 64u, s.opt.fill_waves);
    const uint32_t blocks = (uint32_t)std::min<uint64_t>(slots, std::max<uint64_t>(2, cdiv(chunks, waves)));
    return FillShape{(blocks + 1u) & ~1u, waves * 64u};
}

template <class LaunchOwn>
static void launch_read_kernel(rsq_sim &s, hipStream_t st, const FillShape &shape, size_t lds_bytes, size_t counter_bytes, hipFunction_t spec, void **args, uint32_t *&counters,
                               LaunchOwn &&launch_own) {
    s.cur->fill_counters.reserve(counter_bytes);
    counters = s.cur->fill_counters.as<uint32_t>();
    HIP_CHECK(hipMemsetAsync(counters, 0, counter_bytes, st));
    s.timers["fill_reads"].start(st);
    if (spec) {
        spec_allow_lds(spec, lds_bytes);
        HIP_CHECK(hipModuleLaunchKernel(spec, shape.blocks, 1, 1, shape.threads, 1, 1, (unsigned)lds_bytes, st, args, nullptr));
    } else launch_own();
    s.timers["fill_reads"].stop(st);
    HIP_CHECK(hipGetLastError());
}
template <uint32_t MASK, bool VAR, bool BINNED>
static const uint32_t *launch_fill_kernel(rsq_sim &s, const Fragment *frags, uint64_t n_pairs, uint64_t adapter_first, const RawLayout &raw, hipStream_t st, const FragmentVar *fvars) {
    FillBins bins{};
    if (BINNED)
        bins = build_fill_bins(s, n_pairs, s.dev.n_tiles, st, [&](uint16_t *keys, uint32_t *hist) {
            hipLaunchKernelGGL(k_pair_tiles, dim3(cdiv(n_pairs, kBinBlock)), dim3(kBinBlock), 0, st, s.dev, frags, fvars, n_pairs, adapter_first, keys, hist);
        }, frags, fvars);
    const size_t lds_bytes = fill_lds_bytes(s, MASK != 0, BINNED, &k_fill_reads<MASK, VAR, BINNED>);
    const FillShape shape = fill_shape(s, lds_bytes, n_pairs, 2, fill_block(VAR));
    uint32_t *sizes = s.cur->sizes.as<uint32_t>(), *counters = nullptr;
    RawLayout raw_arg = raw;
    void *args[] = {&s.dev, &s.names, &frags, &n_pairs, &adapter_first, &raw_arg, &sizes, &counters, &fvars, &bins};
    launch_read_kernel(s, st, shape, lds_bytes, 8, spec_kernel(s, SpecKind::kReads, MASK, VAR, BINNED), args, counters, [&] {
        hipLaunchKernelGGL((k_fill_reads<MASK, VAR, BINNED>), dim3(shape.blocks), dim3(shape.threads), lds_bytes, st, s.dev, s.names, frags, n_pairs, adapter_first, raw, sizes, counters, fvars,
                           bins);
    });
    return bins.perm;
}
template <uint32_t MASK, bool VAR = false>
static const uint32_t *launch_fill_mask(rsq_sim &s, const Fragment *frags, uint64_t n_pairs, uint64_t adapter_first, const RawLayout &raw, hipStream_t st, const FragmentVar *fvars = nullptr) {
    if constexpr (MASK != 0)
        if (fill_is_binned(s)) return launch_fill_kernel<MASK, VAR, true>(s, frags, n_pairs, adapter_first, raw, st, fvars);
// ... 348 lines not shown
        SieveRun &r = run[p];
        uint64_t *mail = s.mailbox + 8 * p;
        if (has_slots[p]) sieve_collect(s, r, mail, s_sieve);
        const uint64_t n = has_slots[p] ? r.total : 0;
        const Fragment *frags = s.cur->frags.as<Fragment>();
        const FragmentVar *fvars = nullptr;
        if (n) {
            sieve_emit(s, r, s_sieve);
            frags = s.cur->frags.as<Fragment>();
            fvars = 2 == vm ? s.cur->fvars.as<FragmentVar>() : nullptr;
            if (frags_out) {
                if (frags_cap < total_pairs + n) {
                    g_last_error = "fragment buffer too small: need at least " + std::to_string(total_pairs + n) + " records";
                    return RSQ_ENOSPC;
                }
                HIP_CHECK(hipMemcpyAsync(frags_out + total_pairs, frags, n * sizeof(Fragment), hipMemcpyDeviceToDevice, s_sieve));
            }
            if (parts > 1) {
                HIP_CHECK(hipEventRecord(s.ev_emit, s_sieve));
                HIP_CHECK(hipStreamWaitEvent(s_reads, s.ev_emit, 0));
                if (k >= 2) HIP_CHECK(hipStreamWaitEvent(s_reads, s.cur->text_done, 0));
            }
            const ReadsDone rd = reads_stage(s, frags, n, 0, s_reads, fvars);
            if (parts > 1) {
                HIP_CHECK(hipEventRecord(s.ev_fill, s_reads));
                HIP_CHECK(hipStreamWaitEvent(s_text, s.ev_fill, 0));
            }
            text_stage(s, frags, n, 0, rd, r1, r1_cap, r2, r2_cap, k, s_text, fvars);
        } else {
            HIP_CHECK(hipMemcpyAsync(s.totals.as<uint64_t>() + 2 * (k + 1), s.totals.as<uint64_t>() + 2 * k, 16, hipMemcpyDeviceToDevice, s_text));
        }
        if (parts > 1) HIP_CHECK(hipEventRecord(s.cur->text_done, s_text));
        total_pairs += n;
        if (k + 1 < parts) {
            s.cur = &s.ws[p ^ 1u];
            if (n) HIP_CHECK(hipStreamWaitEvent(s_sieve, s.ev_fill, 0));
            if (k >= 1) HIP_CHECK(hipStreamWaitEvent(s_sieve, s.cur->text_done, 0));
            has_slots[p ^ 1u] = sieve_launch(s, run[p ^ 1u], part_range(k + 1).first, part_range(k + 1).second, s.mailbox + 8 * (p ^ 1u), s_sieve);
        }
    }
    *n_pairs = total_pairs;
    const int rc = total_pairs ? finish_call(s, parts, s.has_variants, r1, r1_cap, r1_len, r2, r2_cap, r2_len, s_text) : (int)RSQ_OK;
    if (total_pairs && (rc == RSQ_OK || rc == RSQ_ENOSPC) && (uint32_t)s.mailbox[5]) s.format_record_bytes = (uint32_t)s.mailbox[5] + 8u;
    if (parts > 1) {
        HIP_CHECK(hipStreamSynchronize(s_sieve));
        HIP_CHECK(hipStreamSynchronize(s_text));
        HIP_CHECK(hipStreamSynchronize(s_reads));
    } else HIP_CHECK(hipStreamSynchronize(st));
    abort_guard.armed = false;
    return rc;
}

RSQ_HD uint32_t error_model_record_size(const ReadMeta &m, uint32_t id_len) { return 1u + id_len + 1u + m.cigar_chars + 2u + digits_u32(m.num_errors) + 1u + 2u * m.read_len + 4u; }
struct RecordIds {
    const char *chars;
    const uint64_t *off;
    const uint32_t *at, *len;
    RSQ_HD const char *begin(uint64_t i) const { return chars + (off ? off[i] : (uint64_t)at[i] + 1u); }
    RSQ_HD uint32_t length(uint64_t i) const { return off ? (uint32_t)(off[i + 1] - off[i]) : len[i]; }
};
__global__ void __launch_bounds__(256) k_record_text_sizes(RawLayout raw, uint64_t n, RecordIds ids, uint32_t *sizes) {
    const uint64_t row = (uint64_t)blockIdx.x * blockDim.x + threadIdx.x;
    if (row >= n) return;
    const uint64_t i = raw.item_of(row);
    sizes[i] = error_model_record_size(raw.meta[row], ids.length(i));
}
template <bool PERM>
__global__ void __launch_bounds__(64) k_record_text_waves(RawLayout raw, uint64_t n, RecordIds ids, const uint64_t *offsets, char *dst, uint64_t cap, uint32_t lds_bytes) {
    extern __shared__ __attribute__((aligned(16))) char s_text[];
    constexpr uint32_t kLineParts = 32u / kFormatRecords;
    const uint32_t lane = threadIdx.x, rec = lane & (kFormatRecords - 1u), part = lane / kFormatRecords, sub = part % kLineParts;
    const bool is_qual = part >= kLineParts;
    const uint64_t first = (uint64_t)blockIdx.x * kFormatRecords;
    if (first >= n || offsets[n] > cap) return;
    const uint64_t last = first + kFormatRecords < n ? first + kFormatRecords : n, row = first + rec;
    const bool active = row < last;
    const uint64_t item = PERM ? (active ? raw.order[row] : 0u) : row;
    const uint64_t g_begin = PERM ? (active ? offsets[item] : 0u) : offsets[first], g_end = PERM ? (active ? offsets[item + 1u] : 0u) : offsets[last];
    const uint32_t skew = (uint32_t)((uint64_t)(uintptr_t)(dst + g_begin) & 15u), bytes = (uint32_t)(g_end - g_begin);
    const uint32_t slot = (lds_bytes / kFormatRecords) & ~15u;
    const bool through_lds = PERM ? __all(skew + bytes <= slot) != 0 : skew + bytes <= lds_bytes;
    ReadMeta m{};
    if (active) m = raw.meta[row];
    const WordColumn seq = raw.seq_of(active ? row : 0u), qual = raw.qual_of(active ? row : 0u), ops = raw.ops_of(active ? row : 0u);
    auto header = [&](auto &t) {
        t.ch('@');
        t.str(ids.begin(item), ids.length(item));
        t.ch(' ');
        cigar_replay(ops, m, t);
        t.str(" E", 2);
        t.num((uint32_t)m.num_errors);
        t.ch('\n');
    };
    if (!through_lds) {
        if (active && part == 0u) {
            WordSinkT<char *> t(dst + offsets[item]);
            header(t);
            format_line(seq, m.read_len, false, t);
            format_line(qual, m.read_len, true, t);
            t.finish();
        }
        return;
    }
    const uint32_t slot_at = PERM ? rec * slot : 0u;
    if (active) {
        RSQ_LDS char *rec_text = (RSQ_LDS char *)s_text + slot_at + skew + (PERM ? 0u : (uint32_t)(offsets[item] - g_begin));
        const uint32_t head = (uint32_t)(offsets[item + 1u] - offsets[item]) - 2u * m.read_len - 4u;
        const uint32_t all_words = (m.read_len + 3u) >> 2, per = (all_words + kLineParts - 1u) / kLineParts, first_word = sub * per;
        const uint32_t line_at = head + (is_qual ? m.read_len + 3u : 0u), part_at = part == 0u ? 0u : line_at + (4u * first_word < m.read_len ? 4u * first_word : m.read_len);
        WordSinkT<RSQ_LDS char *> t(rec_text + part_at);
        if (part == 0u) header(t);
        format_line_part(is_qual ? qual : seq, m.read_len, is_qual, first_word, per, sub == kLineParts - 1u, t);
        t.finish();
    }
    __syncthreads();
    const uint32_t lo = skew, hi = skew + bytes;
    char *g_chunk0 = dst + g_begin - skew;
    const char *s_from = s_text + slot_at;
    for (uint32_t c = (PERM ? part : lane) * 16u; c < hi; c += (PERM ? 64u / kFormatRecords : 64u) * 16u) {
        if (c >= lo && c + 16u <= hi) *reinterpret_cast<uint4 *>(g_chunk0 + c) = *reinterpret_cast<const uint4 *>(s_from + c);
        else
            for (uint32_t b = c < lo ? lo : c; b < c + 16u && b < hi; ++b) g_chunk0[b] = s_from[b];
    }
}

__global__ void __launch_bounds__(256) k_error_model_rows(RawLayout raw, uint64_t n, uint8_t *seq_out, uint8_t *qual_out, uint32_t out_stride) {
    const uint64_t row = ((uint64_t)blockIdx.x * blockDim.x + threadIdx.x) >> 4;
    if (row >= n) return;
    const uint64_t i = raw.item_of(row);
    const uint32_t read_len = raw.meta[row].read_len, nb = read_len < out_stride ? read_len : out_stride;
    const WordColumn seq = raw.seq_of(row), qual = raw.qual_of(row);
    uint32_t *so = reinterpret_cast<uint32_t *>(seq_out + i * out_stride), *qo = reinterpret_cast<uint32_t *>(qual_out + i * out_stride);
    for (uint32_t w = threadIdx.x & 15u; 4u * w < nb; w += 16u) {
        so[w] = seq.at(w);
        qo[w] = qual.at(w);
    }
}

__global__ void k_error_model_out(RawLayout raw, uint64_t n, uint8_t *seq_out, uint8_t *qual_out, uint32_t out_stride, uint16_t *read_len_out, uint16_t *num_errors_out,
                                  uint16_t *tile_out, char *cigar_out, uint32_t cigar_stride, uint32_t *overflow) {
    const uint64_t row = (uint64_t)blockIdx.x * blockDim.x + threadIdx.x;
    if (row >= n) return;
    const uint64_t i = raw.item_of(row);
    const ReadMeta m = raw.meta[row];
    read_len_out[i] = m.read_len;
    num_errors_out[i] = m.num_errors;
    tile_out[i] = m.tile_id;
    const uint32_t nb = m.read_len < out_stride ? m.read_len : out_stride;
    const WordColumn seq = raw.seq_of(row), qual = raw.qual_of(row);
    if ((out_stride | (uint32_t)(uintptr_t)seq_out | (uint32_t)(uintptr_t)qual_out) & 3u)
        for (uint32_t k = 0; k < nb; ++k) {
            seq_out[i * out_stride + k] = (uint8_t)(seq.at(k >> 2) >> (8u * (k & 3u)));
            qual_out[i * out_stride + k] = (uint8_t)(qual.at(k >> 2) >> (8u * (k & 3u)));
        }
    if (m.cigar_chars + 1u > cigar_stride || m.read_len > out_stride) {
        *overflow = 1;
        cigar_out[i * cigar_stride] = 0;
        return;
    }
    TextSink t{cigar_out + i * cigar_stride, 0};
    cigar_replay(raw.ops_of(row), m, t);
    t.ch(0);
}

}

struct FragmentLengthOutside : rsq::Error {
    using rsq::Error::Error;
};
template <class F>
static int guard(F &&f) {
    try {
        return f();
    } catch (const HipError &e) {
        g_last_error = e.what();
        return RSQ_EHIP;
    } catch (const FragmentLengthOutside &e) {
        g_last_error = e.what();
        return RSQ_EIO;
    } catch (const Error &e) {
        g_last_error = e.what();
        return RSQ_EINVAL;
    } catch (const std::exception &e) {
        g_last_error = e.what();
        return RSQ_EINVAL;
    }
}
#define REQUIRE(cond, msg)          \
    do {                            \
        if (!(cond)) {              \
            g_last_error = msg;     \
            return RSQ_EINVAL;      \
        }                           \
    } while (0)

extern "C" {

const char *rsq_last_error(void) { return g_last_error.c_str(); }
const char *rsq_last_warning(void) { return g_last_warning.c_str(); }
const char *rsq_version(void) { return "reseq_amd 0.1 (gfx950)"; }
int rsq_set_option(const char *name, int64_t value) {
    REQUIRE(name, "null argument");
    if (set_option(name, value)) return RSQ_OK;
    g_last_error = std::string("unknown option '") + name + "' (options: " + option_names() + ")";
    return RSQ_EINVAL;
}
int rsq_get_option(const char *name, int64_t *value) {
    REQUIRE(name && value, "null argument");
    if (get_option(name, value)) return RSQ_OK;
    g_last_error = std::string("unknown option '") + name + "' (options: " + option_names() + ")";
    return RSQ_EINVAL;
}

int rsq_device_count(void) {
    int n = 0;
    if (hipGetDeviceCount(&n) != hipSuccess || n <= 0) {
        g_last_error = "no HIP device visible; this library has no CPU fallback";
        return RSQ_ENODEV;
    }
    return n;
}

int rsq_partition_blocks(uint32_t total_blocks, uint32_t workers, const double *weights, uint32_t *bounds) {
    REQUIRE(workers >= 1 && bounds && (weights || !total_blocks), "null argument or no worker");
    double total = 0.0;
    for (uint32_t b = 0; b < total_blocks; ++b) total += weights[b];
    bounds[0] = 1;
    double acc = 0.0;
    uint32_t b = 0;
    for (uint32_t r = 1; r < workers; ++r) {
        const double target = total * (double)r / (double)workers;
        while (b < total_blocks && acc + weights[b] / 2 <= target) acc += weights[b++];
        bounds[r] = b + 1u;
    }
    bounds[workers] = total_blocks + 1u;
    return RSQ_OK;
// ... 395 lines not shown
        return;
    }
    FragmentSrc src;
    src.words = hap_words(S, allele);
    src.word_off = S.seq_word_off[seq];
    src.first = pos;
    src.len = n;
    src.reverse = reversed;
    src.sys_ = nullptr;
    src.converted = nullptr;
    src.gc_prefix = nullptr;
    for (uint32_t w = 0; w < words; ++w) tmpl[w] = 0;
    for (uint32_t k = 0; k < n; ++k) tmpl[k >> 5] |= (uint64_t)src.ref(k) << ((k & 31u) * 2u);
}
int rsq_sim_reference_sequence(rsq_sim *s, uint32_t seq, uint32_t start_pos, uint32_t frag_length, int reversed, int32_t first_variant_id, uint32_t first_variant_pos, uint32_t allele,
                               uint8_t *out, size_t cap) {
    REQUIRE(s && out && s->has_ref && seq < s->dev.n_seqs, "null argument, a simulator without a reference, or no such sequence");
    REQUIRE(allele < (s->has_variants ? s->num_alleles : 1u), "no such allele");
    REQUIRE(frag_length <= (1u << 20) && cap >= frag_length, "room for fewer bases than asked for (at most 2^20 per call)");
    const uint32_t L = s->seq_len[seq];
    REQUIRE(reversed ? start_pos <= L : start_pos < L || 0 == frag_length, "start position outside the sequence");
    if (2 != s->variants_mode)
        REQUIRE(reversed ? frag_length <= start_pos : frag_length <= L - start_pos, "the stretch asked for leaves the sequence");
    if (first_variant_pos) {
        REQUIRE(2 == s->variants_mode, "a start inside inserted bases needs variants with insertions");
        const uint32_t n_var = s->var_ptr[seq + 1] - s->var_ptr[seq];
        REQUIRE(first_variant_id >= 0 && (uint32_t)first_variant_id < n_var && first_variant_pos <= s->variants[s->var_ptr[seq] + first_variant_id].len,
                "first_variant does not name bases of a variant of this sequence");
    }
    if (!frag_length) return RSQ_OK;
    return guard([&] {
        HIP_CHECK(hipSetDevice(s->device));
        const uint32_t words = (frag_length + 31u) / 32u;
        uint64_t *dev = nullptr;
        HIP_CHECK(hipMalloc(&dev, (size_t)(words + 1u) * sizeof(uint64_t)));
        std::vector<uint64_t> host(words + 1u, 0);
        hipError_t e = hipMemset(dev, 0, (size_t)(words + 1u) * sizeof(uint64_t));
        if (e == hipSuccess) {
            hipLaunchKernelGGL(k_reference_sequence, dim3(1), dim3(64), 0, nullptr, s->dev, seq, allele, start_pos, VarStart{first_variant_id, first_variant_pos}, frag_length, reversed != 0,
                               dev, words, reinterpret_cast<uint32_t *>(dev + words));
            e = hipGetLastError();
        }
        if (e == hipSuccess) e = hipMemcpy(host.data(), dev, host.size() * sizeof(uint64_t), hipMemcpyDeviceToHost);
        (void)hipFree(dev);
        HIP_CHECK(e);
        if (host[words]) {
            g_last_error = "the stretch asked for leaves the allele's sequence";
            return RSQ_EINVAL;
        }
        for (uint32_t k = 0; k < frag_length; ++k) out[k] = (uint8_t)((host[k >> 5] >> ((k & 31u) * 2u)) & 3u);
        return RSQ_OK;
    });
}
int rsq_sim_export_reference(rsq_sim *s, const char *path) {
    REQUIRE(s && path, "null argument");
    return guard([&] {
        HIP_CHECK(hipSetDevice(s->device));
        HIP_CHECK(hipDeviceSynchronize());
        export_reference(*s, s->up, path);
        return RSQ_OK;
    });
}
int rsq_sim_import_reference(rsq_sim *s, const char *path) {
    REQUIRE(s && path, "null argument");
    return guard([&] {
        HIP_CHECK(hipSetDevice(s->device));
        MappedFile m(path);
        import_reference(*s, s->up, m.data, m.size, path);
        return RSQ_OK;
    });
}
int rsq_sim_specialize(rsq_sim *s, int kind, int *specialized) {
    REQUIRE(s && specialized && (kind == 0 || kind == 1), "null argument, or a kind that is neither 0 (read pairs) nor 1 (seqToIllumina records)");
    return guard([&] {
        HIP_CHECK(hipSetDevice(s->device));
        const uint32_t mask = effective_fill_mask(s->dev.lds.mask, s->force_fill_mode);
        g_spec_note.clear();
        hipFunction_t fn = spec_kernel(*s, kind == 0 ? SpecKind::kReads : SpecKind::kRecords, mask, kind == 0 && s->has_variants, fill_is_binned(*s));
        if (kind == 1 && fn) fn = spec_kernel(*s, SpecKind::kRecords, mask, true, fill_is_binned(*s));
        *specialized = fn != nullptr;
        if (!s->specialize) g_spec_note = "option specialize is 0: the library's own instantiation of the read kernel runs";
        else if (!mask) g_spec_note = "the read kernel draws in double precision from device memory (no table image): nothing to compile for the profile";
        g_last_warning = g_spec_note;
        return RSQ_OK;
    });
}
int rsq_profile_compile_read_kernel(const rsq_profile *p, int kind, int with_variants, int binned, const char *arch, const char *out_path, size_t *code_bytes, double *seconds) {
    REQUIRE(p && arch && code_bytes && (kind == 0 || kind == 1), "null argument, or a kind that is neither 0 nor 1");
    struct HostArrays : Uploader {
        std::vector<std::unique_ptr<char[]>> owned;
        void *put_bytes(const void *data, size_t bytes) override {
            owned.emplace_back(new char[bytes + 8]);
            memcpy(owned.back().get(), data, bytes);
            return owned.back().get();
        }
        void *put_zeros(size_t bytes) override {
            owned.emplace_back(new char[bytes + 8]());
            return owned.back().get();
        }
        void write_bytes(void *dst, const void *src, size_t bytes) override { memcpy(dst, src, bytes); }
        void read_bytes(void *dst, const void *src, size_t bytes) override { memcpy(dst, src, bytes); }
    };
    int rc = guard([&] {
        HostArrays up;
        SimState s;
        s.prof = p->p;
        pack_tables(s, up);
        pack_profile(s, up);
        if (!s.dev.lds.mask) throw Error("the profile has no table image (" + s.plan_note + "): there is nothing to compile for it");
        const SpecVariant variant{kind == 0 ? SpecKind::kReads : SpecKind::kRecords, s.dev.lds.mask, kind == 0 && with_variants != 0, binned != 0 || s.dev.lds.binned != 0};
        const std::string path = out_path ? out_path : "";
        if (path.size() > 4 && path.compare(path.size() - 4, 4, ".hip") == 0) {
            const std::string program = spec_program(spec_literals(s.dev), variant);
            FILE *f = fopen(out_path, "wb");
            if (!f || fwrite(program.data(), 1, program.size(), f) != program.size()) throw Error(std::string("cannot write ") + out_path);
            fclose(f);
            *code_bytes = program.size();
            if (seconds) *seconds = 0.0;
            return RSQ_OK;
        }
        SpecCode c;
        std::string note;
        if (!spec_compile(s.dev, variant, arch, c, note)) throw Error(note);
        *code_bytes = c.code.size();
        if (seconds) *seconds = c.seconds;
        if (out_path && *out_path) {
            FILE *f = fopen(out_path, "wb");
            if (!f || fwrite(c.code.data(), 1, c.code.size(), f) != c.code.size()) throw Error(std::string("cannot write ") + out_path);
            fclose(f);
        }
        return RSQ_OK;
    });
    return rc;
}
int rsq_set_kernel_cache_dir(const char *path) {
    spec_cache_dir_override() = path ? path : "";
    spec_cache_dir_set() = true;
    return RSQ_OK;
}
int rsq_sim_get_fill_plan(const rsq_sim *s, uint32_t *quality_quads, uint32_t *image_tiles, uint32_t *image_bytes) {
    REQUIRE(s && quality_quads && image_tiles && image_bytes, "null argument");
    *quality_quads = effective_fill_mask(s->dev.lds.mask, s->force_fill_mode);
    *image_tiles = *quality_quads ? s->dev.lds.img_tiles : 0u;
    *image_bytes = *quality_quads ? s->dev.lds.total_words * 4u : 0u;
    return RSQ_OK;
}
int rsq_sim_get_info(const rsq_sim *s, rsq_sim_info *out) {
    REQUIRE(s && out && (s->prepared || s->planned), "simulator not prepared");
    out->total_pairs = s->total_pairs;
    out->adapter_only_pairs = s->adapter_only_pairs;
    out->total_blocks = s->total_blocks;
    out->n_coverage_groups = s->n_groups;
    out->insert_to = s->dev.insert_to;
    out->sys_chain_passes = s->passes;
    out->bias_normalization = s->bias_normalization;
    return RSQ_OK;
}
int rsq_sim_get_thresholds(const rsq_sim *s, double *out, size_t n) {
    REQUIRE(s && out && s->prepared && n == s->thresholds.size(), "bad threshold buffer size");
    memcpy(out, s->thresholds.data(), n * 8);
    return RSQ_OK;
}
int rsq_sim_get_norm_by_len(const rsq_sim *s, double *out, size_t n) {
    REQUIRE(s && out && s->prepared && n == s->norm_by_len.size(), "bad buffer size");
    memcpy(out, s->norm_by_len.data(), n * 8);
    return RSQ_OK;
// ... 1034 lines not shown
```

### reseq_amd/csrc/rsq_spec.h

```cpp
#pragma once
#include <dlfcn.h>
#include <hip/hip_runtime.h>
#include <sys/stat.h>
#include <unistd.h>

#include <chrono>
#include <cstdio>
#include <cstdlib>
#include <cstring>
#include <map>
#include <memory>
#include <mutex>
#include <string>
#include <vector>

#include "rsq_host.h"
#include "rsq_reads.h"

namespace rsq {

#include "build/rsq_embedded.inc"
struct SpecHeader {
    const char *name, *text;
};
constexpr SpecHeader kSpecHeaders[] = {{"rsq_types.h", kSrc_rsq_types_h}, {"rsq_core.h", kSrc_rsq_core_h}, {"rsq_variants.h", kSrc_rsq_variants_h},
                                       {"rsq_text.h", kSrc_rsq_text_h},   {"rsq_reads.h", kSrc_rsq_reads_h}};
constexpr int kSpecHeaderCount = sizeof(kSpecHeaders) / sizeof(kSpecHeaders[0]);

struct Hiprtc {
    using Program = void *;
    int (*create)(Program *, const char *, const char *, int, const char *const *, const char *const *) = nullptr;
    int (*compile)(Program, int, const char *const *) = nullptr;
    int (*log_size)(Program, size_t *) = nullptr;
    int (*log)(Program, char *) = nullptr;
    int (*code_size)(Program, size_t *) = nullptr;
    int (*code)(Program, char *) = nullptr;
    int (*destroy)(Program *) = nullptr;
    int (*version)(int *, int *) = nullptr;
    bool ok = false;
    std::string path;
    std::string comgr;
    static const Hiprtc &get() {
        static Hiprtc h = [] {
            Hiprtc r;
            void *lib = nullptr;
            const bool by_name = options().hiprtc_by_name != 0;
            for (const char *name : {"/opt/rocm/lib/libhiprtc.so", "libhiprtc.so", "libhiprtc.so.7", "libhiprtc.so.6"}) {
                if (by_name && name[0] == '/') continue;
                if ((lib = dlopen(name, RTLD_NOW | RTLD_LOCAL))) break;
            }
            if (!lib && by_name) lib = dlopen("/opt/rocm/lib/libhiprtc.so", RTLD_NOW | RTLD_LOCAL);
            if (!lib) return r;
            auto bind = [&](auto &f, const char *name) { f = reinterpret_cast<std::remove_reference_t<decltype(f)>>(dlsym(lib, name)); return f != nullptr; };
            int bound = 0;
            bound += bind(r.create, "hiprtcCreateProgram") + bind(r.compile, "hiprtcCompileProgram") + bind(r.log_size, "hiprtcGetProgramLogSize") + bind(r.log, "hiprtcGetProgramLog");
            bound += bind(r.code_size, "hiprtcGetCodeSize") + bind(r.code, "hiprtcGetCode") + bind(r.destroy, "hiprtcDestroyProgram") + bind(r.version, "hiprtcVersion");
            r.ok = bound == 8;
            Dl_info info;
            if (r.ok && dladdr(reinterpret_cast<void *>(r.create), &info) && info.dli_fname) {
                char real[4096];
                r.path = realpath(info.dli_fname, real) ? real : info.dli_fname;
            }
            if (r.ok) {
                void *comgr = nullptr;
                for (const char *name : {"libamd_comgr.so.3", "libamd_comgr.so.2", "libamd_comgr.so"}) {
                    if ((comgr = dlopen(name, RTLD_NOW | RTLD_NOLOAD))) break;
                }
                if (!comgr)
                    for (const char *name : {"libamd_comgr.so.3", "libamd_comgr.so.2", "libamd_comgr.so"}) {
                        if ((comgr = dlopen(name, RTLD_NOW | RTLD_LOCAL))) break;
                    }
                void *sym = comgr ? dlsym(comgr, "amd_comgr_get_version") : nullptr;
                if (sym && dladdr(sym, &info) && info.dli_fname) {
                    char real[4096];
                    r.comgr = realpath(info.dli_fname, real) ? real : info.dli_fname;
                }
            }
            return r;
        }();
        return h;
    }
};

inline uint64_t fnv1a(const void *p, size_t n, uint64_t h = 0xcbf29ce484222325ull) {
    const unsigned char *c = static_cast<const unsigned char *>(p);
    for (size_t i = 0; i < n; ++i) h = (h ^ c[i]) * 0x100000001b3ull;
    return h;
}
inline uint64_t fnv1a(const std::string &s, uint64_t h) { return fnv1a(s.data(), s.size(), h); }

inline std::string spec_literals(const DevSim &d) {
    static_assert(sizeof(LdsPlan) % 4 == 0 && std::is_trivially_copyable<LdsPlan>::value, "LdsPlan is a list of 32-bit words");
    std::string t = "namespace rsq { namespace spec {\nconstexpr LdsPlan lds = {";
    uint32_t words[sizeof(LdsPlan) / 4];
    memcpy(words, &d.lds, sizeof(LdsPlan));
    for (size_t i = 0; i < sizeof(LdsPlan) / 4; ++i) t += (i ? ", " : "") + std::to_string(words[i]) + "u";
    t += "};\n";
    t += "constexpr uint32_t n_tiles = " + std::to_string(d.n_tiles) + "u, phred_offset = " + std::to_string((unsigned)d.phred_offset) + "u, max_len_deletion = " +
         std::to_string((unsigned)d.max_len_deletion) + "u, force_exact = " + std::to_string(d.force_exact) + "u;\n";
    t += "} }\n";
    return t;
}

enum class SpecKind : int { kReads = 0, kRecords = 1 };
struct SpecVariant {
    SpecKind kind;
    uint32_t mask;
    bool var, binned;
    int key() const { return ((int)kind << 2) | ((int)var << 1) | (int)binned; }
};
inline const char *spec_kernel_name(SpecKind k) { return k == SpecKind::kReads ? "rsq_spec_fill_reads" : "rsq_spec_fill_records"; }

inline std::string spec_program(const std::string &literals, const SpecVariant &v) {
    std::string t = "#define RSQ_SPEC 1\n#include \"rsq_types.h\"\n" + literals + "#include \"rsq_reads.h\"\nusing namespace rsq;\n";
    const std::string m = std::to_string(v.mask) + "u, ";
    if (v.kind == SpecKind::kReads)
        t += std::string("extern \"C\" __global__ void __launch_bounds__(fill_block(") + (v.var ? "true" : "false") + ")) rsq_spec_fill_reads(DevSim S, NameTable names, const Fragment *frags, uint64_t n_pairs, uint64_t adapter_only_first, "
             "RawLayout raw, uint32_t *sizes, uint32_t *chunk_counters, const FragmentVar *fvars, FillBins bins) {\n    fill_reads_body<" + m + (v.var ? "true, " : "false, ") +
             (v.binned ? "true" : "false") + ">(S, names, frags, n_pairs, adapter_only_first, raw, sizes, chunk_counters, fvars, bins);\n}\n";
    else
        t += "extern \"C\" __global__ void __launch_bounds__(kFillBlockWalk) rsq_spec_fill_records(DevSim S, RecordJob job, RawLayout raw, uint32_t *chunk_counters, FillBins bins) {\n"
             "    fill_records_body<" + m + (v.binned ? "true, " : "false, ") + (v.var ? "true" : "false") + ">(S, job, raw, chunk_counters, bins);\n}\n";
    return t;
}

inline std::string &spec_cache_dir_override() {
    static std::string dir;
    return dir;
}
inline bool &spec_cache_dir_set() {
    static bool set = false;
    return set;
}
inline std::string spec_cache_dir() {
    if (spec_cache_dir_set()) {
        if (!spec_cache_dir_override().empty()) mkdir(spec_cache_dir_override().c_str(), 0755);
        return spec_cache_dir_override();
    }
    const char *x = getenv("XDG_CACHE_HOME"), *h = getenv("HOME");
    std::string base = x && *x ? x : (h && *h ? std::string(h) + "/.cache" : "");
    if (base.empty()) return "";
    mkdir(base.c_str(), 0755);
    base += "/reseq_amd";
    mkdir(base.c_str(), 0755);
    return base;
}

inline std::vector<std::string> spec_extra_options() {
    std::vector<std::string> out;
    const char *e = getenv("RSQ_SPEC_OPTIONS");
    if (!e) return out;
    std::string cur;
    for (const char *p = e;; ++p) {
        if (*p == ' ' || *p == '\0') {
            if (!cur.empty()) out.push_back(cur);
            cur.clear();
            if (!*p) break;
        } else cur += *p;
    }
    return out;
}

struct SpecCode {
    std::vector<char> code;
    std::string cache_path;
    double seconds = 0.0;
    bool from_cache = false;
    int rtc_major = 0, rtc_minor = 0;
};
inline bool spec_compile(const DevSim &dev, const SpecVariant &v, const std::string &arch, SpecCode &out, std::string &note) {
    const Hiprtc &rtc = Hiprtc::get();
    if (!rtc.ok) {
        note = "libhiprtc not found: the read kernels run in the library's own instantiation (not compiled for this profile)";
        return false;
    }
    const std::string literals = spec_literals(dev), program = spec_program(literals, v);
    rtc.version(&out.rtc_major, &out.rtc_minor);
    const char *headers[kSpecHeaderCount], *names[kSpecHeaderCount];
    for (int i = 0; i < kSpecHeaderCount; ++i) headers[i] = kSpecHeaders[i].text, names[i] = kSpecHeaders[i].name;
    uint64_t h = fnv1a(program + " " + std::to_string(RSQ_FILL_BLOCK) + " " + std::to_string(RSQ_FILL_BLOCK_WALK) + " " + std::to_string(RSQ_SCREEN_BATCH) + " " + std::to_string(RSQ_CHUNK_LARGE)
#if defined(RSQ_TRACE_FILL)
// ... 117 lines not shown
```

### reseq_amd/csrc/rsq_text.h

```cpp
#pragma once
#include "rsq_core.h"

namespace rsq {

struct WordColumn {
    uint32_t *p;
    uint64_t pitch;
    RSQ_HD uint32_t &at(uint32_t w) const { return p[(uint64_t)w * pitch]; }
};

template <class Sink>
RSQ_HD void cigar_replay(const WordColumn &ops, const ReadMeta &m, Sink &sink) {
    if (m.plain) {
        if (m.n_iter_m) sink.element('M', m.n_iter_m);
        if (m.n_iter_s) sink.element('S', m.n_iter_s);
        if (m.hard_clip) sink.element('H', m.hard_clip);
        return;
    }
    uint32_t it = 0;
    for (int part = 0; part < 2; ++part) {
        const char base = part ? 'S' : 'M';
        const uint32_t n = part ? m.n_iter_s : m.n_iter_m;
        char element = base;
        uint32_t length = 0;
// ... 120 lines not shown
            *p = (char)(acc & 0xFFu);
            p += 1;
            acc >>= 8;
            --pending;
            --lead;
        }
        if (!lead && pending >= 4u) {
            *reinterpret_cast<typename WordPtr<P>::type>(p) = (uint32_t)acc;
            p += 4;
            acc >>= 32;
            pending -= 4u;
        }
    }
    RSQ_HD void ch(char c) { push((uint8_t)c, 1u); }
    RSQ_HD void bytes(uint32_t word, uint32_t count) { push(count < 4u ? word & ((1u << (8u * count)) - 1u) : word, count); }
    RSQ_HD void finish() {
        while (pending) {
            *p = (char)(acc & 0xFFu);
            p += 1;
            acc >>= 8;
            --pending;
        }
    }
};

RSQ_HD uint32_t digits_u32(uint32_t v) {
    uint32_t n = 1;
    while (v >= 10u) {
        v /= 10u;
        ++n;
    }
    return n;
}
RSQ_HD uint32_t digits_u64(uint64_t v) {
    if (v <= 0xFFFFFFFFull) return digits_u32((uint32_t)v);
    uint32_t n = 1;
    while (v >= 10) {
        v /= 10;
        ++n;
    }
    return n;
}


template <class Sink>
RSQ_HD void format_header(const DevSim &S, const NameTable &names, bool has_f, const Fragment &f, uint64_t adapter_only_number, const ReadMeta &m, const WordColumn &ops, Sink &t,
                          bool has_fv, const FragmentVar &fv) {
    t.ch('@');
    t.str(names.base_identifier, names.base_len);
    if (has_f) {
        const uint32_t end = has_fv ? fv.end : f.start + f.len;
        t.num(f.block);
        t.ch('_');
        t.num(f.number);
        if (1u < S.num_alleles) {
            t.str("_allele", 7);
            t.num((uint32_t)f.allele);
        }
        t.ch(':');
        t.num(f.strand ? end : f.start + 1u);
        t.ch(':');
        t.str(names.names + names.name_ptr[f.seq], names.name_ptr[f.seq + 1] - names.name_ptr[f.seq]);
        t.ch(':');
        t.num(f.strand ? f.start + 1u : end);
    } else {
        t.ch('0');
        t.ch('_');
        t.num(adapter_only_number);
        t.str(":0:Adapter:0", 12);
    }
    t.ch(':');
    t.num((uint32_t)S.tiles[m.tile_id]);
    t.str(":1337:1337 ", 11);
    cigar_replay(ops, m, t);
    t.str(" E", 2);
    t.num((uint32_t)m.num_errors);
    t.ch('\n');
}
template <class Sink>
RSQ_HD void format_header(const DevSim &S, const NameTable &names, const Fragment *f, uint64_t adapter_only_number, const ReadMeta &m, const WordColumn &ops, Sink &t,
                          const FragmentVar *fv = nullptr) {
    format_header(S, names, f != nullptr, f ? *f : Fragment{}, adapter_only_number, m, ops, t, fv != nullptr, fv ? *fv : FragmentVar{});
}
RSQ_HD uint32_t base_letters(uint32_t codes) {
#if defined(__HIP_DEVICE_COMPILE__)
    return __builtin_amdgcn_perm(0x4E4E4E4Eu, 0x54474341u, codes);
#else
    uint32_t out = 0;
    for (uint32_t k = 0; k < 4u; ++k) {
        const uint32_t b = (codes >> (8u * k)) & 0xFFu;
        out |= (uint32_t)("ACGTN"[b < 4u ? b : 4u]) << (8u * k);
    }
    return out;
#endif
}
template <class Sink>
RSQ_HD void format_line_part(const WordColumn &row, uint32_t read_len, bool is_qual, uint32_t first_word, uint32_t n_words, bool with_end, Sink &t) {
    const uint32_t all_words = (read_len + 3u) >> 2, end_word = first_word + n_words < all_words ? first_word + n_words : all_words;
    constexpr uint32_t kAhead = 10u;
    for (uint32_t i = first_word; i < end_word; i += kAhead) {
        uint32_t w[kAhead];
#pragma unroll
        for (uint32_t k = 0; k < kAhead; ++k) w[k] = i + k < end_word ? row.at(i + k) : 0u;
#pragma unroll
        for (uint32_t k = 0; k < kAhead; ++k) {
            const uint32_t at = 4u * (i + k);
            if (i + k >= end_word) break;
            const uint32_t left = read_len - at, text = is_qual ? w[k] : base_letters(w[k]);
            if (left >= 4u) t.push(text, 4u);
            else t.push(text & ((1u << (8u * left)) - 1u), left);
        }
    }
    if (with_end) {
        if (is_qual) t.push('\n', 1u);
        else t.push('\n' | ('+' << 8) | ('\n' << 16), 3u);
    }
}
template <class Sink>
RSQ_HD void format_line(const WordColumn &row, uint32_t read_len, bool is_qual, Sink &t) {
    format_line_part(row, read_len, is_qual, 0u, (read_len + 3u) >> 2, true, t);
}
template <class P>
RSQ_HD uint32_t format_record(const DevSim &S, const NameTable &names, bool has_f, const Fragment &f, uint64_t adapter_only_number, const ReadMeta &m, const WordColumn &seq,
                              const WordColumn &qual, const WordColumn &ops, P dst, bool has_fv, const FragmentVar &fv) {
    WordSinkT<P> t(dst);
    format_header(S, names, has_f, f, adapter_only_number, m, ops, t, has_fv, fv);
    format_line(seq, m.read_len, false, t);
    format_line(qual, m.read_len, true, t);
    t.finish();
    return t.n;
}
template <class P>
RSQ_HD uint32_t format_record(const DevSim &S, const NameTable &names, const Fragment *f, uint64_t adapter_only_number, const ReadMeta &m, const WordColumn &seq,
                              const WordColumn &qual, const WordColumn &ops, P dst, const FragmentVar *fv = nullptr) {
    return format_record(S, names, f != nullptr, f ? *f : Fragment{}, adapter_only_number, m, seq, qual, ops, dst, fv != nullptr, fv ? *fv : FragmentVar{});
}

RSQ_HD uint32_t record_size(const DevSim &S, const NameTable &names, bool has_f, const Fragment &f, uint64_t adapter_only_number, const ReadMeta &m, bool has_fv, const FragmentVar &fv) {
    uint32_t n = 1u + names.base_len;
    if (has_f) {
        const uint32_t end = has_fv ? fv.end : f.start + f.len;
        if (1u < S.num_alleles) n += 7u + digits_u64(f.allele);
        n += digits_u64(f.block) + 1u + digits_u64(f.number) + 1u + digits_u64(f.strand ? end : f.start + 1u) + 1u +
             (names.name_ptr[f.seq + 1] - names.name_ptr[f.seq]) + 1u + digits_u64(f.strand ? f.start + 1u : end);
    } else n += 2u + digits_u64(adapter_only_number) + 12u;
    n += 1u + digits_u64(S.tiles[m.tile_id]) + 11u + m.cigar_chars + 2u + digits_u64(m.num_errors) + 1u;
    return n + 2u * m.read_len + 4u;
}
RSQ_HD uint32_t record_size(const DevSim &S, const NameTable &names, const Fragment *f, uint64_t adapter_only_number, const ReadMeta &m, const FragmentVar *fv = nullptr) {
    return record_size(S, names, f != nullptr, f ? *f : Fragment{}, adapter_only_number, m, fv != nullptr, fv ? *fv : FragmentVar{});
}

}
```

### reseq_amd/csrc/rsq_types.h

```cpp
#pragma once
#if defined(__HIPCC_RTC__)
using __hip_internal::int32_t;
using __hip_internal::int64_t;
using __hip_internal::uint16_t;
using __hip_internal::uint32_t;
using __hip_internal::uint64_t;
using __hip_internal::uint8_t;
typedef unsigned long uintptr_t;
#define RSQ_DEVICE_BUILD 1
#define RSQ_HD __host__ __device__ __forceinline__
#elif defined(__HIPCC__)
#include <stdint.h>
#include <hip/hip_runtime.h>
#define RSQ_DEVICE_BUILD 1
#define RSQ_HD __host__ __device__ __forceinline__
#else
#include <stdint.h>
#define RSQ_DEVICE_BUILD 0
#define RSQ_HD inline
#endif

namespace rsq {

constexpr uint32_t kBlockSize = 1000;
constexpr uint32_t kSurBlocks = 3;
constexpr uint32_t kSurRange = 10;
constexpr uint32_t kSurStart = 10;
constexpr uint32_t kSurSize = 1u << 20;
constexpr uint32_t kSqFragmentLengthBinSize = 10;

enum : uint32_t { kDomSieve = 1, kDomPair = 2, kDomSysErr = 3, kDomErrModel = 4, kDomReplaceN = 5, kDomRefBias = 6, kDomMethylation = 7 };

struct DevTable {
    uint32_t k;
    uint32_t par0_off;
    uint32_t from[4];
    uint32_t rows[4];
    uint32_t off[4];
    uint32_t max_value;
    uint32_t off32;
    uint32_t f32_ok;
    uint32_t sure_range;
};
static_assert(sizeof(DevTable) == 72, "descriptor layout");
static_assert(__builtin_offsetof(DevTable, par0_off) == 4, "lds_stage_descriptors rewrites word 1 of a descriptor");
constexpr uint32_t kNoLds = 0xFFFFFFFFu;
#ifndef RSQ_CHUNK_LARGE
#define RSQ_CHUNK_LARGE 4
#endif
constexpr uint32_t kChunkSmall = 3, kChunkLarge = RSQ_CHUNK_LARGE;
RSQ_HD uint32_t chunk_pairs(uint32_t k) { return k <= 2u * kChunkSmall ? kChunkSmall : kChunkLarge; }
RSQ_HD uint32_t chunks_of(uint32_t k, uint32_t u) { return (k + 2u * u - 1u) / (2u * u); }
RSQ_HD uint32_t row_stride(uint32_t k) {
    const uint32_t u = chunk_pairs(k), kp = chunks_of(k, u) * 2u * u;
    return (kp & 2u) ? kp : kp + 2u;
}
RSQ_HD uint32_t quads_of(uint32_t k) { return (k + 3u) / 4u; }
RSQ_HD uint32_t row_slot32(uint32_t quads) {
    const uint32_t w = quads * 4u;
    return (w & 4u) ? w : w + 4u;
}
constexpr uint32_t kQuadsSmall = 2, kSlotSmall = 8;
constexpr uint32_t kQualityQuads[] = {3, 6, 10, 11, 12};
constexpr uint32_t kChainQuads[] = {8, 16, 26};
constexpr uint32_t kRingSlots = 2, kRingLag = 1;
constexpr uint32_t kRingRows = kRingSlots + 1u;

struct FamilyGeo {
    uint32_t from[4];
    uint32_t last[4];
    uint32_t before[4];
    uint32_t table_rows;
    uint32_t off32;
    uint32_t lds;
    uint32_t lds_rows;
    uint32_t lds_stride;
    uint32_t lds2;
    uint32_t lds2_stride;
    uint32_t values;
    uint32_t values_src;
};

struct LdsPlan {
    uint32_t mask;
    uint32_t img_tiles;
    uint32_t binned;
    uint32_t desc_words;
    uint32_t par0_words;
    uint32_t par0_indel_bytes;
    uint32_t slot_q, slot_b, slot_i;
    uint32_t quads_q;
    uint32_t rate_rows_q, rate_rows_b;
    uint32_t q3_off, b3_off;
    uint32_t q3_stride, b3_stride;
    uint32_t ring_off, ring_stride;
    uint32_t total_words;
    FamilyGeo q, b, i;
};

struct Fragment {
    uint32_t seq;
    uint32_t start;
    uint32_t len;
    uint16_t dup;
    uint8_t strand;
    uint8_t allele;
    uint32_t block;
    uint32_t number;
};

struct ReadMeta {
    uint16_t read_len;
    uint16_t num_errors;
    uint16_t n_iter_m;
    uint16_t n_iter_s;
    uint16_t hard_clip;
    uint16_t tile_id;
    uint16_t cigar_chars;
    uint16_t plain;
};

struct DevVariant {
    uint32_t pos;
    uint32_t len;
    uint32_t off;
    uint32_t pad;
    uint64_t allele[2];
};
struct AlleleVar {
    uint32_t pos;
    uint32_t vid;
    int32_t shift;
    int32_t gc;
};
struct FragmentVar {
    uint32_t end;
    uint32_t sub;
    int32_t start_var;
    uint32_t start_var_pos;
    int32_t end_var;
    uint32_t end_var_pos;
};
struct ExtraStart {
    uint32_t pos;
    uint32_t sub;
    int32_t first_variant_id;
    uint32_t start_variant_pos;
};

struct DevAdapters {
    uint32_t n;
    const uint8_t *seqs;
    const uint32_t *seq_ptr;
    const uint16_t *sys;
    const double *adapter_cp;
    const double *cut_cp;
    const uint32_t *cut_ptr;
    const uint32_t *cut_from;
};

struct DevReadLengths {
    uint32_t fixed;
    uint32_t to;
    uint32_t row_first;
    uint32_t rows;
    const uint32_t *row_ptr;
    const uint32_t *row_from;
    const uint64_t *values;
};

struct DevSim {
    uint64_t seed;
    const double *pool;
    const uint32_t *chain_sure;
    const float *pool32;
    const uint8_t *par0;
    const DevTable *quality;
    const DevTable *seq_quality;
    const DevTable *base_call;
    const DevTable *dom_error;
    const DevTable *error_rate;
    const DevTable *indels;
    LdsPlan lds;
    uint32_t force_exact;
    uint32_t chain_quads;
    uint32_t n_tiles;
    uint8_t phred_offset;
    uint16_t max_len_deletion;
    uint32_t reset_distance;
    uint16_t sys_gc_range;
    const double *tile_cp;
    const uint16_t *tiles;
    DevAdapters adapters[2];
    DevReadLengths read_lengths[2];
    const double *polya_cp;
    uint32_t polya_n, polya_from;
    double overrun_cp[4];
    const uint64_t *insert_lengths;
    uint32_t n_seqs;
    const uint64_t *ref_words;
    const uint32_t *gc_prefix;
    const uint64_t *seq_word_off;
    const uint32_t *seq_len;
    const uint64_t *seq_base_off;
    const uint16_t *sys_fwd;
    const uint16_t *sys_rev;
    uint32_t num_alleles;
    uint32_t variants_loaded;
    uint64_t hap_stride;
    const DevVariant *variants;
    const uint32_t *var_ptr;
    const uint8_t *var_bases;
    const uint32_t *var_bases_gc;
    const AlleleVar *allele_map;
    const uint32_t *allele_map_ptr;
    const uint16_t *var_err_fwd, *var_err_rev;
    uint32_t *walk_error;
    const ExtraStart *extra;
    const uint32_t *block_extra_ptr;
    uint32_t insert_from;
    uint32_t insert_to;
    const double *thresholds;
    const double *gap_q;
    const uint32_t *gap_seg_end;
    const uint32_t *coverage_group;
    const double *ref_seq_bias;
    const double *insert_lengths_bias;
    const double *gc_bias;
    const double *sur_bias;
    double dispersion[2];
    double bias_normalization;
    uint32_t total_blocks;
    const uint32_t *block_seq;
    const uint32_t *first_block;
    const uint32_t *meth_ptr;
    const uint32_t *meth_first, *meth_second;
    const double *meth_rate;
};

#if defined(RSQ_SPEC)
#define RSQ_PLAN(S, field) (::rsq::spec::lds.field)
#define RSQ_SIM(S, field) (::rsq::spec::field)
#else
#define RSQ_PLAN(S, field) ((S).lds.field)
#define RSQ_SIM(S, field) ((S).field)
#endif

struct NameTable {
    const char *names;
    const uint32_t *name_ptr;
    char base_identifier[64];
    uint32_t base_len;
};

}
```

Measured before the change: 229.0 million.

## Pack base and quality into one byte code per position in raw read arrays

Replaces the separate raw sequence and quality word arrays with a single code array. Each position stores quality*mul+base, using a multiplier chosen from the profile's quality and base ranges (8, 5, or a 16-bit wide fallback). The generate kernel writes and the format/copy kernels read about half as many bytes for read contents. In exchange, decoding adds per-word unpack arithmetic (multiply-shift division for the mul=5 code), and a new host helper and API are added to check the encoding.

```diff
diff --git a/include/reseq_amd.h b/include/reseq_amd.h
--- a/include/reseq_amd.h
+++ b/include/reseq_amd.h
@@ -41,6 +41,8 @@
 int rsq_profile_remove_indel_errors(rsq_profile *p);
 int rsq_profile_max_read_length(const rsq_profile *p, uint32_t *out);
 int rsq_profile_num_tiles(const rsq_profile *p, uint32_t *out);
+int rsq_profile_base_code(const rsq_profile *p, uint32_t *mul);
+int rsq_base_code_lines(uint32_t mul, uint32_t phred_offset, const uint8_t *bases, const uint8_t *quals, uint32_t n, char *seq_line, char *qual_line);
 int rsq_profile_max_len_deletion(const rsq_profile *p, uint32_t *out);
 int rsq_profile_ref_seq_bias(const rsq_profile *p, double *out, size_t cap, size_t *n);
 
diff --git a/reseq_amd/api.py b/reseq_amd/api.py
--- a/reseq_amd/api.py
+++ b/reseq_amd/api.py
@@ -81,6 +81,8 @@
     "rsq_sim_get_sequence_lengths": (C.c_int, [_vp, _vp, _sz, C.POINTER(_u32)]),
     "rsq_sim_import_reference": (C.c_int, [_vp, C.c_char_p]),
     "rsq_set_kernel_cache_dir": (C.c_int, [C.c_char_p]),
+    "rsq_profile_base_code": (C.c_int, [_vp, C.POINTER(_u32)]),
+    "rsq_base_code_lines": (C.c_int, [_u32, _u32, _vp, _vp, _u32, _vp, _vp]),
     "rsq_profile_compile_read_kernel": (C.c_int, [_vp, C.c_int, C.c_int, C.c_int, C.c_char_p, C.c_char_p, C.POINTER(C.c_size_t), C.POINTER(C.c_double)]),
     "rsq_sim_get_thresholds": (C.c_int, [_vp, _vp, _sz]),
     "rsq_sim_get_norm_by_len": (C.c_int, [_vp, _vp, _sz]),
@@ -224,6 +226,11 @@
         _check(lib().rsq_profile_compile_read_kernel(self.h, kind, int(with_variants), int(binned), arch.encode(), os.fsencode(out_path) if out_path else None, C.byref(n), C.byref(t)))
         return n.value, t.value
 
+    def base_code(self):
+        v = C.c_uint32()
+        _check(lib().rsq_profile_base_code(self.h, C.byref(v)))
+        return v.value
+
     def change_error_rate(self, multiplier):
         _check(lib().rsq_profile_change_error_rate(self.h, multiplier))
 
@@ -242,6 +249,14 @@
         if self.h:
             lib().rsq_profile_free(self.h)
             self.h = C.c_void_p()
+
+
+def base_code_lines(mul, phred_offset, bases, quals):
+    bases, quals = np.ascontiguousarray(bases, np.uint8), np.ascontiguousarray(quals, np.uint8)
+    n = len(bases)
+    seq, qual = C.create_string_buffer(n + 8), C.create_string_buffer(n + 8)
+    _check(lib().rsq_base_code_lines(mul, phred_offset, bases.ctypes.data, quals.ctypes.data, n, seq, qual))
+    return seq.raw[:n + 3], qual.raw[:n + 1]
 
 
 def load_profile(path, ipf_path=None, ipf_precision=5.0):
diff --git a/reseq_amd/csrc/rsq_core.h b/reseq_amd/csrc/rsq_core.h
--- a/reseq_amd/csrc/rsq_core.h
+++ b/reseq_amd/csrc/rsq_core.h
@@ -726,7 +726,7 @@
             if (!insertion) ++org_pos;
         }
         if (!deletion) {
-            out.put(par.read_pos, put_base, q + RSQ_SIM(S, phred_offset));
+            out.put(par.read_pos, put_base, q, RSQ_SIM(S, code_mul), RSQ_SIM(S, phred_offset));
             par.last_written_qual = q;
             ++par.read_pos;
         }
diff --git a/reseq_amd/csrc/rsq_format.h b/reseq_amd/csrc/rsq_format.h
--- a/reseq_amd/csrc/rsq_format.h
+++ b/reseq_amd/csrc/rsq_format.h
@@ -202,10 +202,10 @@
         if (frags) f = frags[pair];
         if (frags && fvars) fv = fvars[pair];
     }
-    const WordColumn seq = raw.seq_of(r), qual = raw.qual_of(r), ops = raw.ops_of(r);
+    const WordColumn codes = raw.codes_of(r), ops = raw.ops_of(r);
     const uint64_t ao_number = adapter_only_first + pair + 1u;
     if (!through_lds) {
-        if (active && part == 0u) format_record(S, names, frags != nullptr, f, ao_number, m, seq, qual, ops, dst + offsets[pair], frags && fvars, fv);
+        if (active && part == 0u) format_record(S, names, frags != nullptr, f, ao_number, m, codes, raw.code, ops, dst + offsets[pair], frags && fvars, fv);
         return;
     }
     const uint32_t slot_at = PERM ? rec * kSlot : 0u;
@@ -217,7 +217,7 @@
         const uint32_t part_at = part == 0u ? 0u : line_at + (4u * first_word < m.read_len ? 4u * first_word : m.read_len);
         WordSinkT<RSQ_LDS char *> t(rec_text + part_at);
         if (part == 0u) format_header(S, names, frags != nullptr, f, ao_number, m, ops, t, frags && fvars, fv);
-        format_line_part(is_qual ? qual : seq, m.read_len, is_qual, first_word, per, sub == kLineParts - 1u, t);
+        format_line_part(codes, raw.code, m.read_len, is_qual, first_word, per, sub == kLineParts - 1u, t);
         t.finish();
     }
     __syncthreads();
diff --git a/reseq_amd/csrc/rsq_pack.h b/reseq_amd/csrc/rsq_pack.h
--- a/reseq_amd/csrc/rsq_pack.h
+++ b/reseq_amd/csrc/rsq_pack.h
@@ -445,11 +445,27 @@
 
 inline uint32_t effective_fill_mask(uint32_t plan_mask, int forced) { return forced == 0 ? 0u : plan_mask; }
 
+inline uint32_t profile_code_mul(const Profile &p) {
+    uint32_t max_quality = 1, max_base = 3;
+    for (const HostTable &t : p.quality)
+        for (uint32_t v : t.par0) max_quality = std::max(max_quality, v);
+    for (const HostTable &t : p.base_call)
+        for (uint32_t v : t.par0) max_base = std::max(max_base, v);
+    for (const HostTable &t : p.indels)
+        for (uint32_t v : t.par0) max_base = std::max(max_base, v >= 2u ? v - 2u : 0u);
+    const uint32_t mul = base_code_mul(max_quality, max_base);
+    if (!mul || max_quality + p.phred_offset > 255u)
+        throw Error("the profile's qualities (up to " + std::to_string(max_quality) + " above phred offset " + std::to_string((unsigned)p.phred_offset) + ") or base values (up to " +
+                    std::to_string(max_base) + ") are outside every code of the raw array (quality + phred offset is one character)");
+    return mul;
+}
+
 inline void pack_profile(SimState &s, Uploader &up) {
     const Profile &p = s.prof;
     DevSim &d = s.dev;
     d.n_tiles = p.n_tiles();
     d.phred_offset = p.phred_offset;
+    d.code_mul = (uint16_t)profile_code_mul(p);
     d.max_len_deletion = p.max_len_deletion;
     d.reset_distance = p.reset_distance;
     d.tile_cp = up.put(discrete_cp(p.tile_abundance.data(), p.tile_abundance.size()));
diff --git a/reseq_amd/csrc/rsq_reads.h b/reseq_amd/csrc/rsq_reads.h
--- a/reseq_amd/csrc/rsq_reads.h
+++ b/reseq_amd/csrc/rsq_reads.h
@@ -6,18 +6,36 @@
 namespace rsq {
 
 struct ReadOut {
-    WordColumn seq, qual, ops;
+    WordColumn codes, ops;
     uint32_t cur_word, cur_index;
-    uint32_t seq_word, qual_word, n_put;
-    RSQ_HD void put(uint32_t pos, uint32_t base, uint32_t qual_char) {
-        const uint32_t sh = (pos & 3u) * 8u;
-        seq_word |= base << sh;
-        qual_word |= qual_char << sh;
+    uint32_t code_word, n_put;
+#if !RSQ_DEVICE_BUILD
+    WordColumn qual_row = WordColumn{nullptr, 0};
+    uint32_t qual_word = 0;
+#endif
+    RSQ_HD void put(uint32_t pos, uint32_t base, uint32_t quality, uint32_t mul, uint32_t phred_offset) {
+        uint32_t code = quality * mul + base;
+        bool wide = mul == kCodeWide;
+#if !RSQ_DEVICE_BUILD
+        if (qual_row.p) {
+            uint32_t bases, quals;
+            BaseCode{mul, phred_offset}.unpack_first(code, bases, quals);
+            qual_word |= ((quals + phred_offset) & 0xFFu) << ((pos & 3u) * 8u);
+            if ((pos & 3u) == 3u) {
+                qual_row.at(pos >> 2) = qual_word;
+                qual_word = 0;
+            }
+            code = bases;
+            wide = false;
+        }
+#endif
+        (void)phred_offset;
+        const uint32_t per = wide ? 1u : 3u, bits = wide ? 16u : 8u, word = wide ? pos >> 1 : pos >> 2;
+        code_word |= code << ((pos & per) * bits);
         n_put = pos + 1u;
-        if ((pos & 3u) == 3u) {
-            seq.at(pos >> 2) = seq_word;
-            qual.at(pos >> 2) = qual_word;
-            seq_word = qual_word = 0;
+        if ((pos & per) == per) {
+            codes.at(word) = code_word;
+            code_word = 0;
         }
     }
     RSQ_HD void op(uint32_t it, uint32_t code) {
@@ -29,18 +47,40 @@
         }
         cur_word |= code << ((it & 15u) * 2u);
     }
-    RSQ_HD void finish() {
+    RSQ_HD void finish(bool wide = false) {
         ops.at(cur_index) = cur_word;
-        if (n_put & 3u) {
-            seq.at(n_put >> 2) = seq_word;
-            qual.at(n_put >> 2) = qual_word;
-        }
-    }
-};
-RSQ_HD ReadOut make_read_out(const WordColumn &seq, const WordColumn &qual, const WordColumn &ops) { return ReadOut{seq, qual, ops, 0u, 0u, 0u, 0u, 0u}; }
+#if !RSQ_DEVICE_BUILD
+        if (qual_row.p) {
+            wide = false;
+            if (n_put & 3u) qual_row.at(n_put >> 2) = qual_word;
+        }
+#endif
+        if (n_put & (wide ? 1u : 3u)) codes.at(wide ? n_put >> 1 : n_put >> 2) = code_word;
+    }
+};
+RSQ_HD ReadOut make_read_out(const WordColumn &codes, const WordColumn &ops) { return ReadOut{codes, ops, 0u, 0u, 0u, 0u}; }
+#if !RSQ_DEVICE_BUILD
+inline ReadOut make_read_out(const WordColumn &seq, const WordColumn &qual, const WordColumn &ops) {
+    ReadOut out = make_read_out(seq, ops);
+    out.qual_row = qual;
+    return out;
+}
+template <class P>
+inline uint32_t format_record(const DevSim &S, const NameTable &names, const Fragment *f, uint64_t adapter_only_number, const ReadMeta &m, const WordColumn &seq,
+                              const WordColumn &qual, const WordColumn &ops, P dst, const FragmentVar *fv = nullptr) {
+    uint32_t *codes = new uint32_t[m.read_len / 2u + 2u](), ops_unused[2] = {0u, 0u};
+    ReadOut packed = make_read_out(WordColumn{codes, 1}, WordColumn{ops_unused, 1});
+    for (uint32_t k = 0; k < m.read_len; ++k)
+        packed.put(k, (seq.at(k >> 2) >> (8u * (k & 3u))) & 0xFFu, ((qual.at(k >> 2) >> (8u * (k & 3u))) - S.phred_offset) & 0xFFu, S.code_mul, S.phred_offset);
+    packed.finish(S.code_mul == kCodeWide);
+    const uint32_t n = format_record(S, names, f, adapter_only_number, m, WordColumn{codes, 1}, BaseCode{S.code_mul, S.phred_offset}, ops, dst, fv);
+    delete[] codes;
+    return n;
+}
+#endif
 
 struct RawLayout {
-    uint32_t *seq, *qual;
+    uint32_t *codes;
     uint32_t *ops;
     ReadMeta *meta;
     uint64_t pitch;
@@ -48,10 +88,10 @@
     uint32_t template_words;
     const uint32_t *order;
     RSQ_HD uint64_t item_of(uint64_t row) const { return order ? order[row] : row; }
-    RSQ_HD WordColumn seq_of(uint64_t r) const { return WordColumn{seq + r, pitch}; }
-    RSQ_HD WordColumn qual_of(uint64_t r) const { return WordColumn{qual + r, pitch}; }
+    BaseCode code;
+    RSQ_HD WordColumn codes_of(uint64_t r) const { return WordColumn{codes + r, pitch}; }
     RSQ_HD WordColumn ops_of(uint64_t r) const { return WordColumn{ops + r, pitch}; }
-    RSQ_HD ReadOut out_of(uint64_t r) const { return make_read_out(seq_of(r), qual_of(r), ops_of(r)); }
+    RSQ_HD ReadOut out_of(uint64_t r) const { return make_read_out(codes_of(r), ops_of(r)); }
 };
 
 struct FragmentSrc {
@@ -887,7 +927,7 @@
     }
     if (active) {
         m.finalize(meta);
-        out.finish();
+        out.finish(RSQ_SIM(S, code_mul) == kCodeWide);
     }
 }
 
diff --git a/reseq_amd/csrc/rsq_sim.hip b/reseq_amd/csrc/rsq_sim.hip
--- a/reseq_amd/csrc/rsq_sim.hip
+++ b/reseq_amd/csrc/rsq_sim.hip
@@ -192,7 +192,7 @@
     struct Workspace {
         DevBuf fvars;
         DevBuf slot_table;
-        DevBuf counts, offsets, tile_sums, scan_total, frags, raw_seq, raw_qual, raw_ops, raw_meta, sizes, off_r1, off_r2, fill_counters, hits, hit_count, cands, pairs_of, pair_off, templates, rec_flags, rec_index, rec_count;
+        DevBuf counts, offsets, tile_sums, scan_total, frags, raw_codes, raw_ops, raw_meta, sizes, off_r1, off_r2, fill_counters, hits, hit_count, cands, pairs_of, pair_off, templates, rec_flags, rec_index, rec_count;
         DevBuf bin_keys, bin_small, bin_perm, bin_frags, bin_fvars;
         DevBuf fa_counts, fa_first, fa_at, fa_len, fa_id_len, fa_frag_len, fa_seg, fa_codes, fa_summary;
         DevBuf cell_info;
@@ -450,11 +450,10 @@
 
 static RawLayout raw_layout(rsq_sim &s, uint64_t n_reads) {
     const uint64_t pitch = (n_reads + 63u) & ~(uint64_t)63u;
-    s.cur->raw_seq.reserve((uint64_t)(s.read_stride / 4u) * pitch * 4 + 16);
-    s.cur->raw_qual.reserve((uint64_t)(s.read_stride / 4u) * pitch * 4 + 16);
+    s.cur->raw_codes.reserve((uint64_t)(s.read_stride / 4u) * (s.dev.code_mul == kCodeWide ? 2u : 1u) * pitch * 4 + 16);
     s.cur->raw_ops.reserve((uint64_t)s.ops_stride * pitch * 4 + 16);
     s.cur->raw_meta.reserve(n_reads * sizeof(ReadMeta) + 16);
-    return RawLayout{s.cur->raw_seq.as<uint32_t>(), s.cur->raw_qual.as<uint32_t>(), s.cur->raw_ops.as<uint32_t>(), s.cur->raw_meta.as<ReadMeta>(), pitch, nullptr, 0, nullptr};
+    return RawLayout{s.cur->raw_codes.as<uint32_t>(), s.cur->raw_ops.as<uint32_t>(), s.cur->raw_meta.as<ReadMeta>(), pitch, nullptr, 0, nullptr, BaseCode{s.dev.code_mul, s.dev.phred_offset}};
 }
 
 template <class CountKernel>
@@ -969,7 +968,7 @@
     const bool through_lds = PERM ? __all(skew + bytes <= slot) != 0 : skew + bytes <= lds_bytes;
     ReadMeta m{};
     if (active) m = raw.meta[row];
-    const WordColumn seq = raw.seq_of(active ? row : 0u), qual = raw.qual_of(active ? row : 0u), ops = raw.ops_of(active ? row : 0u);
+    const WordColumn codes = raw.codes_of(active ? row : 0u), ops = raw.ops_of(active ? row : 0u);
     auto header = [&](auto &t) {
         t.ch('@');
         t.str(ids.begin(item), ids.length(item));
@@ -983,8 +982,8 @@
         if (active && part == 0u) {
             WordSinkT<char *> t(dst + offsets[item]);
             header(t);
-            format_line(seq, m.read_len, false, t);
-            format_line(qual, m.read_len, true, t);
+            format_line(codes, raw.code, m.read_len, false, t);
+            format_line(codes, raw.code, m.read_len, true, t);
             t.finish();
         }
         return;
@@ -997,7 +996,7 @@
         const uint32_t line_at = head + (is_qual ? m.read_len + 3u : 0u), part_at = part == 0u ? 0u : line_at + (4u * first_word < m.read_len ? 4u * first_word : m.read_len);
         WordSinkT<RSQ_LDS char *> t(rec_text + part_at);
         if (part == 0u) header(t);
-        format_line_part(is_qual ? qual : seq, m.read_len, is_qual, first_word, per, sub == kLineParts - 1u, t);
+        format_line_part(codes, raw.code, m.read_len, is_qual, first_word, per, sub == kLineParts - 1u, t);
         t.finish();
     }
     __syncthreads();
@@ -1016,11 +1015,14 @@
     if (row >= n) return;
     const uint64_t i = raw.item_of(row);
     const uint32_t read_len = raw.meta[row].read_len, nb = read_len < out_stride ? read_len : out_stride;
-    const WordColumn seq = raw.seq_of(row), qual = raw.qual_of(row);
+    const WordColumn codes = raw.codes_of(row);
     uint32_t *so = reinterpret_cast<uint32_t *>(seq_out + i * out_stride), *qo = reinterpret_cast<uint32_t *>(qual_out + i * out_stride);
     for (uint32_t w = threadIdx.x & 15u; 4u * w < nb; w += 16u) {
-        so[w] = seq.at(w);
-        qo[w] = qual.at(w);
+        const uint32_t left = read_len - 4u * w, keep = left >= 4u ? 0xFFFFFFFFu : (1u << (8u * left)) - 1u;
+        uint32_t bases, quals;
+        raw.code.load(codes, w, bases, quals);
+        so[w] = bases & keep;
+        qo[w] = (quals + raw.code.offset * 0x01010101u) & keep;
     }
 }
 
@@ -1034,11 +1036,13 @@
     num_errors_out[i] = m.num_errors;
     tile_out[i] = m.tile_id;
     const uint32_t nb = m.read_len < out_stride ? m.read_len : out_stride;
-    const WordColumn seq = raw.seq_of(row), qual = raw.qual_of(row);
+    const WordColumn codes = raw.codes_of(row);
     if ((out_stride | (uint32_t)(uintptr_t)seq_out | (uint32_t)(uintptr_t)qual_out) & 3u)
         for (uint32_t k = 0; k < nb; ++k) {
-            seq_out[i * out_stride + k] = (uint8_t)(seq.at(k >> 2) >> (8u * (k & 3u)));
-            qual_out[i * out_stride + k] = (uint8_t)(qual.at(k >> 2) >> (8u * (k & 3u)));
+            uint32_t bases, quals;
+            raw.code.load(codes, k >> 2, bases, quals);
+            seq_out[i * out_stride + k] = (uint8_t)(bases >> (8u * (k & 3u)));
+            qual_out[i * out_stride + k] = (uint8_t)((quals >> (8u * (k & 3u))) + raw.code.offset);
         }
     if (m.cigar_chars + 1u > cigar_stride || m.read_len > out_stride) {
         *overflow = 1;
@@ -1600,6 +1604,32 @@
         if (!s->specialize) g_spec_note = "option specialize is 0: the library's own instantiation of the read kernel runs";
         else if (!mask) g_spec_note = "the read kernel draws in double precision from device memory (no table image): nothing to compile for the profile";
         g_last_warning = g_spec_note;
+        return RSQ_OK;
+    });
+}
+int rsq_profile_base_code(const rsq_profile *p, uint32_t *mul) {
+    REQUIRE(p && mul, "null argument");
+    return guard([&] {
+        *mul = profile_code_mul(p->p);
+        return RSQ_OK;
+    });
+}
+int rsq_base_code_lines(uint32_t mul, uint32_t phred_offset, const uint8_t *bases, const uint8_t *quals, uint32_t n, char *seq_line, char *qual_line) {
+    REQUIRE(bases && quals && seq_line && qual_line && (mul == kCodeNarrow || mul == kCodeGeneral || mul == kCodeWide) && phred_offset <= 255u, "null argument, or a multiplier that is no code");
+    return guard([&] {
+        std::vector<uint32_t> codes(n / 2u + 2u, 0u), ops(2u, 0u);
+        ReadOut out = make_read_out(WordColumn{codes.data(), 1}, WordColumn{ops.data(), 1});
+        for (uint32_t k = 0; k < n; ++k) {
+            if (!base_code_holds(mul, quals[k], bases[k])) throw Error("a base or a quality outside what the code holds");
+            out.put(k, bases[k], quals[k], mul, phred_offset);
+        }
+        out.finish(mul == kCodeWide);
+        const BaseCode code{mul, phred_offset};
+        WordSinkT<char *> s(seq_line), q(qual_line);
+        format_line(WordColumn{codes.data(), 1}, code, n, false, s);
+        s.finish();
+        format_line(WordColumn{codes.data(), 1}, code, n, true, q);
+        q.finish();
         return RSQ_OK;
     });
 }
diff --git a/reseq_amd/csrc/rsq_spec.h b/reseq_amd/csrc/rsq_spec.h
--- a/reseq_amd/csrc/rsq_spec.h
+++ b/reseq_amd/csrc/rsq_spec.h
@@ -96,7 +96,7 @@
     memcpy(words, &d.lds, sizeof(LdsPlan));
     for (size_t i = 0; i < sizeof(LdsPlan) / 4; ++i) t += (i ? ", " : "") + std::to_string(words[i]) + "u";
     t += "};\n";
-    t += "constexpr uint32_t n_tiles = " + std::to_string(d.n_tiles) + "u, phred_offset = " + std::to_string((unsigned)d.phred_offset) + "u, max_len_deletion = " +
+    t += "constexpr uint32_t n_tiles = " + std::to_string(d.n_tiles) + "u, phred_offset = " + std::to_string((unsigned)d.phred_offset) + "u, code_mul = " + std::to_string((unsigned)d.code_mul) + "u, max_len_deletion = " +
          std::to_string((unsigned)d.max_len_deletion) + "u, force_exact = " + std::to_string(d.force_exact) + "u;\n";
     t += "} }\n";
     return t;
diff --git a/reseq_amd/csrc/rsq_text.h b/reseq_amd/csrc/rsq_text.h
--- a/reseq_amd/csrc/rsq_text.h
+++ b/reseq_amd/csrc/rsq_text.h
@@ -226,6 +226,36 @@
                           const FragmentVar *fv = nullptr) {
     format_header(S, names, f != nullptr, f ? *f : Fragment{}, adapter_only_number, m, ops, t, fv != nullptr, fv ? *fv : FragmentVar{});
 }
+struct BaseCode {
+    uint32_t mul;
+    uint32_t offset;
+    RSQ_HD uint32_t recip() const { return mul == kCodeNarrow ? 128u : 205u; }
+    RSQ_HD void split(uint32_t codes, uint32_t &bases, uint32_t &quals) const {
+        if (mul == kCodeNarrow) {
+            bases = codes & 0x07070707u;
+            quals = (codes >> 3) & 0x1F1F1F1Fu;
+            return;
+        }
+        const uint32_t even = ((codes & 0x00FF00FFu) * recip() >> 10) & 0x003F003Fu, odd = (((codes >> 8) & 0x00FF00FFu) * recip() >> 10) & 0x003F003Fu;
+        quals = even | (odd << 8);
+        bases = codes - quals * mul;
+    }
+    RSQ_HD bool wide() const { return mul == kCodeWide; }
+    RSQ_HD void unpack_first(uint32_t code, uint32_t &base, uint32_t &quality) const {
+        if (wide()) {
+            base = code & 0xFFu;
+            quality = (code >> 8) & 0xFFu;
+        } else {
+            split(code & 0xFFu, base, quality);
+        }
+    }
+    RSQ_HD void load(const WordColumn &row, uint32_t i, uint32_t &bases, uint32_t &quals) const {
+        if (!wide()) return split(row.at(i), bases, quals);
+        const uint32_t lo = row.at(2u * i), hi = row.at(2u * i + 1u);
+        bases = (lo & 0xFFu) | ((lo >> 8) & 0xFF00u) | ((hi & 0xFFu) << 16) | ((hi << 8) & 0xFF000000u);
+        quals = ((lo >> 8) & 0xFFu) | ((lo >> 16) & 0xFF00u) | ((hi << 8) & 0xFF0000u) | (hi & 0xFF000000u);
+    }
+};
 RSQ_HD uint32_t base_letters(uint32_t codes) {
 #if defined(__HIP_DEVICE_COMPILE__)
     return __builtin_amdgcn_perm(0x4E4E4E4Eu, 0x54474341u, codes);
@@ -239,18 +269,21 @@
 #endif
 }
 template <class Sink>
-RSQ_HD void format_line_part(const WordColumn &row, uint32_t read_len, bool is_qual, uint32_t first_word, uint32_t n_words, bool with_end, Sink &t) {
+RSQ_HD void format_line_part(const WordColumn &row, const BaseCode &code, uint32_t read_len, bool is_qual, uint32_t first_word, uint32_t n_words, bool with_end, Sink &t) {
     const uint32_t all_words = (read_len + 3u) >> 2, end_word = first_word + n_words < all_words ? first_word + n_words : all_words;
     constexpr uint32_t kAhead = 10u;
     for (uint32_t i = first_word; i < end_word; i += kAhead) {
         uint32_t w[kAhead];
 #pragma unroll
-        for (uint32_t k = 0; k < kAhead; ++k) w[k] = i + k < end_word ? row.at(i + k) : 0u;
+        for (uint32_t k = 0; k < kAhead; ++k) w[k] = i + k < end_word && !code.wide() ? row.at(i + k) : 0u;
 #pragma unroll
         for (uint32_t k = 0; k < kAhead; ++k) {
             const uint32_t at = 4u * (i + k);
             if (i + k >= end_word) break;
-            const uint32_t left = read_len - at, text = is_qual ? w[k] : base_letters(w[k]);
+            uint32_t bases, quals;
+            if (code.wide()) code.load(row, i + k, bases, quals);
+            else code.split(w[k], bases, quals);
+            const uint32_t left = read_len - at, text = is_qual ? quals + code.offset * 0x01010101u : base_letters(bases);
             if (left >= 4u) t.push(text, 4u);
             else t.push(text & ((1u << (8u * left)) - 1u), left);
         }
@@ -261,23 +294,23 @@
     }
 }
 template <class Sink>
-RSQ_HD void format_line(const WordColumn &row, uint32_t read_len, bool is_qual, Sink &t) {
-    format_line_part(row, read_len, is_qual, 0u, (read_len + 3u) >> 2, true, t);
-}
-template <class P>
-RSQ_HD uint32_t format_record(const DevSim &S, const NameTable &names, bool has_f, const Fragment &f, uint64_t adapter_only_number, const ReadMeta &m, const WordColumn &seq,
-                              const WordColumn &qual, const WordColumn &ops, P dst, bool has_fv, const FragmentVar &fv) {
+RSQ_HD void format_line(const WordColumn &row, const BaseCode &code, uint32_t read_len, bool is_qual, Sink &t) {
+    format_line_part(row, code, read_len, is_qual, 0u, (read_len + 3u) >> 2, true, t);
+}
+template <class P>
+RSQ_HD uint32_t format_record(const DevSim &S, const NameTable &names, bool has_f, const Fragment &f, uint64_t adapter_only_number, const ReadMeta &m, const WordColumn &codes,
+                              const BaseCode &code, const WordColumn &ops, P dst, bool has_fv, const FragmentVar &fv) {
     WordSinkT<P> t(dst);
     format_header(S, names, has_f, f, adapter_only_number, m, ops, t, has_fv, fv);
-    format_line(seq, m.read_len, false, t);
-    format_line(qual, m.read_len, true, t);
+    format_line(codes, code, m.read_len, false, t);
+    format_line(codes, code, m.read_len, true, t);
     t.finish();
     return t.n;
 }
 template <class P>
-RSQ_HD uint32_t format_record(const DevSim &S, const NameTable &names, const Fragment *f, uint64_t adapter_only_number, const ReadMeta &m, const WordColumn &seq,
-                              const WordColumn &qual, const WordColumn &ops, P dst, const FragmentVar *fv = nullptr) {
-    return format_record(S, names, f != nullptr, f ? *f : Fragment{}, adapter_only_number, m, seq, qual, ops, dst, fv != nullptr, fv ? *fv : FragmentVar{});
+RSQ_HD uint32_t format_record(const DevSim &S, const NameTable &names, const Fragment *f, uint64_t adapter_only_number, const ReadMeta &m, const WordColumn &codes,
+                              const BaseCode &code, const WordColumn &ops, P dst, const FragmentVar *fv = nullptr) {
+    return format_record(S, names, f != nullptr, f ? *f : Fragment{}, adapter_only_number, m, codes, code, ops, dst, fv != nullptr, fv ? *fv : FragmentVar{});
 }
 
 RSQ_HD uint32_t record_size(const DevSim &S, const NameTable &names, bool has_f, const Fragment &f, uint64_t adapter_only_number, const ReadMeta &m, bool has_fv, const FragmentVar &fv) {
diff --git a/reseq_amd/csrc/rsq_types.h b/reseq_amd/csrc/rsq_types.h
--- a/reseq_amd/csrc/rsq_types.h
+++ b/reseq_amd/csrc/rsq_types.h
@@ -66,6 +66,19 @@
 constexpr uint32_t kRingSlots = 2, kRingLag = 1;
 constexpr uint32_t kRingRows = kRingSlots + 1u;
 
+constexpr uint32_t kCodeNarrow = 8, kCodeGeneral = 5, kCodeWide = 256;
+RSQ_HD bool base_code_holds(uint32_t mul, uint32_t max_quality, uint32_t max_base) {
+    if (mul == kCodeNarrow) return max_quality < 32u && max_base < 8u;
+    if (mul == kCodeGeneral) return max_quality * kCodeGeneral + kCodeGeneral - 1u <= 255u && max_base < kCodeGeneral;
+    return mul == kCodeWide && max_quality <= 255u && max_base < 8u;
+}
+RSQ_HD uint32_t base_code_mul(uint32_t max_quality, uint32_t max_base) {
+    return base_code_holds(kCodeNarrow, max_quality, max_base)    ? kCodeNarrow
+           : base_code_holds(kCodeGeneral, max_quality, max_base) ? kCodeGeneral
+           : base_code_holds(kCodeWide, max_quality, max_base)    ? kCodeWide
+                                                                   : 0u;
+}
+
 struct FamilyGeo {
     uint32_t from[4];
     uint32_t last[4];
@@ -189,6 +202,7 @@
     uint16_t max_len_deletion;
     uint32_t reset_distance;
     uint16_t sys_gc_range;
+    uint16_t code_mul;
     const double *tile_cp;
     const uint16_t *tiles;
     DevAdapters adapters[2];
```

Result: no change. 230.2 million, median of 6 (+0.5%).
